# unibas-gravis/GiNGR

Measured on AMD Instinct MI355X. Metric: GiNGR update iters/sec, 50k<->50k CPD, higher is better.
Workload: dtype f64; 1 GPU; CPD update, synthetic Gaussian clouds 50000<->50000, GPMM rank 100, w=0.1, rigid global transform, sigma2_0=5032.781; points=50000, targets=50000, rank=100, parallelism=row-shard x1, exchange=single shard

## Files before the change

gingr_amd/_native.py:

```python
from __future__ import annotations

import ctypes
import os
from ctypes import POINTER, c_char_p, c_double, c_int, c_int32, c_int64, c_void_p

import numpy as np

_HERE = os.path.dirname(os.path.abspath(__file__))
LIB_PATH = os.environ.get("GINGR_HIP_LIB") or os.path.join(_HERE, "libgingr_hip.so")

GINGR_OK = 0
ERR_BAD_ARGUMENT, ERR_HIP, ERR_NONFINITE, ERR_NOT_SPD, ERR_NO_DEVICE, ERR_STATE = 1, 2, 3, 4, 5, 6
NUM_PHASES = 3
NUM_SEGMENTS = 2
SEGMENT_FULLFIT = 2
SEGMENT_REVSUM = 3
FLAVOUR_CPD, FLAVOUR_ICP, FLAVOUR_ICP_SURFACE = 0, 1, 2
RCCL_UNIQUE_ID_BYTES = 128

_STATUS_NAMES = {
    1: "GINGR_ERR_BAD_ARGUMENT", 2: "GINGR_ERR_HIP", 3: "GINGR_ERR_NONFINITE", 4: "GINGR_ERR_NOT_SPD",
    5: "GINGR_ERR_NO_DEVICE", 6: "GINGR_ERR_STATE",
}


class GingrNativeError(RuntimeError):
    def __init__(self, code: int, where: str, text: str = ""):
        self.code = code
        super().__init__(f"{where}: {_STATUS_NAMES.get(code, code)} {text}".strip())


class StateScalars(ctypes.Structure):
    _fields_ = [
        ("euler", c_double * 3), ("center", c_double * 3), ("translation", c_double * 3),
        ("scale", c_double), ("sigma2", c_double), ("iteration", c_int32), ("status", c_int32),
    ]


class CpdParams(ctypes.Structure):
    _fields_ = [("w", c_double), ("lambda_", c_double)]


class IcpParams(ctypes.Structure):
    _fields_ = [("initial_sigma", c_double), ("end_sigma", c_double), ("max_iterations", c_int32)]


class MhRequest(ctypes.Structure):
    _fields_ = [
        ("flavour", c_int32), ("kind", c_int32), ("cpd", POINTER(CpdParams)), ("icp", POINTER(IcpParams)),
        ("z", POINTER(c_double)), ("alpha", POINTER(c_double)), ("scalars", POINTER(StateScalars)),
        ("eval_sdev", c_double), ("eval_points", c_int64), ("need_forward", c_int32),
    ]


class MhResult(ctypes.Structure):
    _fields_ = [
        ("scalars", StateScalars), ("log_value", c_double), ("dist_sum", c_double), ("dist_max", c_double), ("count", c_int64),
        ("log_q_forward", c_double), ("log_q_backward", c_double), ("forward_status", c_int32), ("backward_status", c_int32),
    ]


ALLREDUCE_FN = ctypes.CFUNCTYPE(c_int, c_void_p, c_int32, c_void_p, c_int64)
_dp = POINTER(c_double)
_ip = POINTER(c_int32)

KERNEL_GAUSSIAN_MIXTURE, KERNEL_DOT, KERNEL_LOOKUP = 0, 1, 2
OPT_CULL, OPT_FINE_CULL, OPT_NN_GRID, OPT_TRI_GRID, OPT_SPLIT_EXCHANGE, OPT_GRAM_DOWNDATE = 0, 1, 2, 3, 4, 5


class ScalarKernel(ctypes.Structure):
    _fields_ = [("kind", c_int32), ("n_kernels", c_int32), ("sigmas", _dp), ("scalings", _dp), ("mirror", c_double),
                ("scaling", c_double), ("lookup", _dp)]


SIGNATURES = {
    "gingr_device_count": (c_int, []),
    "gingr_ctx_create": (c_int, [c_int, POINTER(c_void_p)]),
    "gingr_ctx_destroy": (None, [c_void_p]),
    "gingr_last_error": (c_char_p, [c_void_p]),
    "gingr_ctx_set_stream": (c_int, [c_void_p, c_void_p]),
    "gingr_ctx_get_stream": (c_void_p, [c_void_p]),
    "gingr_ctx_synchronize": (c_int, [c_void_p]),
    "gingr_build_info": (c_char_p, []),
    "gingr_ctx_set_option": (c_int, [c_void_p, c_int32, c_int32]),
    "gingr_ctx_get_option": (c_int, [c_void_p, c_int32, POINTER(c_int32)]),
    "gingr_cpd_stats": (c_int, [c_void_p, c_int64, _dp, c_int64, _dp, c_double, c_double, _dp, _dp, _dp, _dp, _dp]),
    "gingr_cpd_initial_sigma2": (c_int, [c_void_p, c_int64, _dp, c_int64, _dp, _dp]),
    "gingr_nn": (c_int, [c_void_p, c_int64, _dp, c_int64, _dp, _ip, _dp, _dp]),
    "gingr_gauss_block": (c_int, [c_void_p, c_int64, _dp, c_int64, _dp, c_double, c_double, _dp]),
    "gingr_model_upload": (c_int, [c_void_p, c_int64, c_int32, _dp, _dp, _dp, _dp, c_int64, c_int64, POINTER(c_void_p)]),
    "gingr_model_destroy": (None, [c_void_p]),
    "gingr_model_gram_exchange": (c_int, [c_void_p, POINTER(c_void_p), POINTER(c_int64)]),
    "gingr_model_finalize": (c_int, [c_void_p, c_void_p]),
    "gingr_fitter_set_meshes": (c_int, [c_void_p, c_int64, POINTER(c_int32), c_int64, POINTER(c_int32)]),
    "gingr_fitter_set_surface_method": (c_int, [c_void_p, c_int32]),
    "gingr_fitter_set_correspondence_direction": (c_int, [c_void_p, c_int32]),
    "gingr_fitter_get_reversed_correspondence": (c_int, [c_void_p, POINTER(c_int32), _dp]),
    "gingr_fitter_update_icp_surface_async": (c_int, [c_void_p, POINTER(IcpParams), c_int32]),
    "gingr_fitter_set_stop_threshold": (c_int, [c_void_p, c_double]),
    "gingr_fitter_stop_rule_hit": (c_int, [c_void_p, POINTER(c_int32)]),
    "gingr_fitter_icp_surface_phase_async": (c_int, [c_void_p, POINTER(IcpParams), c_int32]),
    "gingr_fitter_get_surface_correspondence": (c_int, [c_void_p, _dp, _dp]),
    "gingr_fitter_surface_distance_stats": (c_int, [c_void_p, c_int32, c_int64, _dp, c_int32, c_double, _dp]),
    "gingr_fitter_mh_step": (c_int, [c_void_p, POINTER(MhRequest), _dp, _dp, POINTER(MhResult)]),
    "gingr_fitter_mh_restore": (c_int, [c_void_p]),
    "gingr_classic_cpd_create": (c_int, [c_void_p, c_int32, c_int64, _dp, c_int64, _dp, c_double, c_double, c_double, POINTER(c_void_p)]),
    "gingr_classic_cpd_destroy": (None, [c_void_p]),
    "gingr_classic_cpd_iterate": (c_int, [c_void_p, c_int32]),
    "gingr_classic_cpd_get": (c_int, [c_void_p, _dp, POINTER(c_double), _dp, _dp]),
    "gingr_classic_cpd_set": (c_int, [c_void_p, _dp, c_double]),
    "gingr_mesh_distance_stats": (c_int, [c_void_p, c_int64, _dp, c_int64, _dp, c_int64, POINTER(c_int32), c_int32, c_double, _dp]),
    "gingr_fitter_update_icp_surface_sample_async": (c_int, [c_void_p, POINTER(IcpParams), _dp]),
    "gingr_fitter_posterior_logpdf_icp_surface": (c_int, [c_void_p, POINTER(IcpParams), _dp, POINTER(c_double)]),
    "gingr_rigid_icp_create": (c_int, [c_void_p, c_int32, c_int64, _dp, c_int64, _dp, POINTER(c_void_p)]),
    "gingr_rigid_icp_destroy": (None, [c_void_p]),
    "gingr_rigid_icp_iterate": (c_int, [c_void_p, c_int32, _dp]),
    "gingr_rigid_icp_get": (c_int, [c_void_p, _dp, _dp]),
    "gingr_rigid_icp_set": (c_int, [c_void_p, _dp]),
    "gingr_fitter_set_fit_points": (c_int, [c_void_p, _dp]),
    "gingr_nicp_solve": (c_int, [c_void_p, c_int32, c_int64, _dp, c_int64, _ip, _dp, _dp, c_int32, _ip, _dp, c_double, c_double, c_double,
                                 _dp, _dp]),
    "gingr_mesh_closest_points": (c_int, [c_void_p, c_int64, _dp, c_int64, _dp, c_int64, _ip, _dp, _dp, _ip, _dp]),
    "gingr_model_new_reference": (c_int, [c_void_p, c_void_p, c_int64, _dp, _ip, _dp, c_int64, c_int64, POINTER(c_void_p)]),
    "gingr_gpmm_build_diagonal": (c_int, [c_void_p, c_int64, _dp, POINTER(ScalarKernel), POINTER(ScalarKernel), POINTER(ScalarKernel),
                                          c_double, c_int32, c_int64, c_int64, POINTER(c_void_p)]),
    "gingr_gpmm_build_gaussian": (c_int, [c_void_p, c_int64, _dp, c_int32, _dp, _dp, c_double, c_int32, c_int64, c_int64,
                                          POINTER(c_void_p)]),
    "gingr_pointset_distance_extrema": (c_int, [c_void_p, _dp, c_int64, _dp, _dp]),
    "gingr_model_download": (c_int, [c_void_p, c_void_p, _dp, _dp, _dp, _dp]),
    "gingr_model_num_points": (c_int64, [c_void_p]),
    "gingr_model_rank": (c_int32, [c_void_p]),
    "gingr_model_instance": (c_int, [c_void_p, c_void_p, _dp, _dp, _dp, _dp, c_double, _dp]),
    "gingr_model_coefficients": (c_int, [c_void_p, c_void_p, _dp, _dp, _dp, _dp, _dp]),
    "gingr_model_posterior_mean": (c_int, [c_void_p, c_void_p, _dp, _dp, _dp, _dp, _dp, c_int32, _ip, _dp, _dp, _dp, _dp]),
    "gingr_fitter_create": (c_int, [c_void_p, c_void_p, POINTER(c_void_p)]),
    "gingr_fitter_destroy": (None, [c_void_p]),
    "gingr_fitter_set_target": (c_int, [c_void_p, c_int64, _dp]),
    "gingr_fitter_set_landmarks": (c_int, [c_void_p, c_int32, _ip, _dp, _dp]),
    "gingr_fitter_set_options": (c_int, [c_void_p, c_int32, c_double]),
    "gingr_fitter_set_state": (c_int, [c_void_p, _dp, POINTER(StateScalars)]),
    "gingr_fitter_get_state": (c_int, [c_void_p, _dp, POINTER(StateScalars), _dp]),
    "gingr_fitter_get_cpd_stats": (c_int, [c_void_p, _dp, _dp, _dp, _dp]),
    "gingr_fitter_get_icp_idx": (c_int, [c_void_p, _ip, _dp]),
    "gingr_fitter_update_cpd_async": (c_int, [c_void_p, POINTER(CpdParams), c_int32]),
    "gingr_fitter_update_icp_async": (c_int, [c_void_p, POINTER(IcpParams), c_int32]),
    "gingr_fitter_update_cpd_sample_async": (c_int, [c_void_p, POINTER(CpdParams), _dp]),
    "gingr_fitter_update_icp_sample_async": (c_int, [c_void_p, POINTER(IcpParams), _dp]),
    "gingr_fitter_posterior_logpdf_cpd": (c_int, [c_void_p, POINTER(CpdParams), _dp, _dp]),
    "gingr_fitter_posterior_logpdf_icp": (c_int, [c_void_p, POINTER(IcpParams), _dp, _dp]),
    "gingr_fitter_retry_counter": (c_int, [c_void_p, c_int32, POINTER(c_int32)]),
# ... 92 lines not shown
```

gingr_amd/csrc/common.h:

```cpp
#pragma once
#include <cstdlib>

#include <hip/hip_runtime.h>

#include <cstdarg>
#include <cstdint>
#include <cstdio>
#include <cstring>
#include <string>
#include <vector>

#include "../../include/gingr_hip.h"

#define GINGR_TIMERS 10

struct gingr_ctx {
    int device = 0;
    hipStream_t own_stream = nullptr;
    hipStream_t stream = nullptr;
    char err[512] = {0};
    bool timing = false;
    struct Span {
        hipEvent_t a, b;
        int which;
    };
    std::vector<Span> spans;
    std::vector<hipEvent_t> pool;
    double t_ms[GINGR_TIMERS] = {0};
    int64_t t_n[GINGR_TIMERS] = {0};
    int cull = 1;
    int tri_grid = 1;
    int nn_grid = 1;
    int32_t *regime_host = nullptr, *regime_dev = nullptr;
    int fine_override = -1;
    unsigned long long *nn_tests = nullptr;
    void *rccl_comm = nullptr;
    int32_t rccl_world = 0, rccl_rank = 0;
    int split_exchange = 0;
    int gram_downdate = -1;
    hipStream_t side_stream = nullptr, exchange_stream = nullptr;
    hipEvent_t split_ev[2] = {nullptr, nullptr};
    void *scratch = nullptr;
    size_t scratch_bytes = 0;
};

int gingr_set_error(gingr_ctx *ctx, int code, const char *fmt, ...);
void gingr_ctx_rccl_release(gingr_ctx *ctx);

#define HIP_TRY(ctx, expr)                                                                                   \
    do {                                                                                                     \
        hipError_t e__ = (expr);                                                                             \
        if (e__ != hipSuccess)                                                                               \
            return gingr_set_error((ctx), GINGR_ERR_HIP, "%s failed: %s (%s:%d)", #expr, hipGetErrorString(e__), \
                                   __FILE__, __LINE__);                                                      \
    } while (0)

#define GINGR_TRY(expr)          \
    do {                         \
        int s__ = (expr);        \
        if (s__ != GINGR_OK) return s__; \
    } while (0)

struct DevBuf {
    void *p = nullptr;
    size_t bytes = 0;
    DevBuf() = default;
    DevBuf(const DevBuf &) = delete;
    DevBuf &operator=(const DevBuf &) = delete;
    ~DevBuf() {
        if (p) (void)hipFree(p);
    }
    hipError_t alloc(size_t n) {
        if (p) (void)hipFree(p);
        p = nullptr;
        bytes = n;
        const hipError_t e = hipMalloc(&p, n ? n : 8);
        static const bool poison = getenv("GINGR_DEBUG_POISON") != nullptr;
        if (e == hipSuccess && poison) {
            (void)hipMemset(p, 0xFF, n ? n : 8);
            (void)hipDeviceSynchronize();
        }
        return e;
    }
    template <typename T>
    T *as() const {
        return reinterpret_cast<T *>(p);
    }
};

void set_dynamic_lds(const void *func, int bytes);
template <typename K>
inline void set_dynamic_lds(K *kern, size_t bytes) {
    set_dynamic_lds(reinterpret_cast<const void *>(kern), (int)bytes);
}

struct TimerScope {
    gingr_ctx *ctx;
    int which;
    hipEvent_t a = nullptr, b = nullptr;
    TimerScope(gingr_ctx *c, int w);
    void stop();
    ~TimerScope();
};

static inline int64_t ceil_div(int64_t a, int64_t b) { return (a + b - 1) / b; }
static inline int64_t round_up(int64_t a, int64_t b) { return ceil_div(a, b) * b; }

struct Cloud {
    const double *x, *y, *z;
    int64_t n;
};

int64_t cpd_colsum_ws_doubles(int64_t M, int64_t N);
int64_t cpd_rowstats_ws_doubles(int64_t M, int64_t N);
int64_t nn_ws_bytes(int64_t M, int64_t N);
bool nn_small_applies(int64_t M, int64_t N);
int64_t nn_small_ws_bytes(int64_t M, int64_t N);
void launch_nn_small(gingr_ctx *ctx, Cloud query, Cloud target, void *ws, int32_t *idx, double *d2);

#define GINGR_AUX 8
void launch_cloud_centroid(gingr_ctx *ctx, Cloud c, double *out3);
// ... 154 lines not shown
```

gingr_amd/csrc/context.hip:

```cpp
#include "common.h"

#include <map>
#include <mutex>
void set_dynamic_lds(const void *func, int bytes) {
    static std::mutex mu;
    static std::map<std::pair<int, const void *>, int> limit;
    int dev = 0;
    (void)hipGetDevice(&dev);
    std::lock_guard<std::mutex> lock(mu);
    int &have = limit[std::make_pair(dev, func)];
    if (have >= bytes) return;
    if (hipFuncSetAttribute(func, hipFuncAttributeMaxDynamicSharedMemorySize, bytes) == hipSuccess)
        have = bytes;
    else
        (void)hipGetLastError();
}


int gingr_set_error(gingr_ctx *ctx, int code, const char *fmt, ...) {
    if (ctx) {
        va_list ap;
        va_start(ap, fmt);
        vsnprintf(ctx->err, sizeof(ctx->err), fmt, ap);
        va_end(ap);
// ... 47 lines not shown
    int n = 0;
    if (hipGetDeviceCount(&n) != hipSuccess) return 0;
    return n;
}

const char *gingr_build_info(void) { return "libgingr_hip gfx950 (CDNA4) f64; built " __DATE__ " " __TIME__; }

int gingr_ctx_create(int device, gingr_ctx **out) {
    if (!out) return GINGR_ERR_BAD_ARGUMENT;
    *out = nullptr;
    int n = 0;
    if (hipGetDeviceCount(&n) != hipSuccess || n <= 0) return GINGR_ERR_NO_DEVICE;
    if (device < 0 || device >= n) return GINGR_ERR_BAD_ARGUMENT;
    if (hipSetDevice(device) != hipSuccess) return GINGR_ERR_HIP;
    gingr_ctx *ctx = new gingr_ctx();
    ctx->device = device;
    if (hipStreamCreateWithFlags(&ctx->own_stream, hipStreamNonBlocking) != hipSuccess) {
        delete ctx;
        return GINGR_ERR_HIP;
    }
    ctx->stream = ctx->own_stream;
    void *hp = nullptr, *dp = nullptr;
    if (hipHostMalloc(&hp, 64, hipHostMallocMapped) == hipSuccess) {
        memset(hp, 0, 64);
        if (hipHostGetDevicePointer(&dp, hp, 0) == hipSuccess) {
            ctx->regime_host = static_cast<int32_t *>(hp);
            ctx->regime_dev = static_cast<int32_t *>(dp);
        } else {
            (void)hipHostFree(hp);
        }
    }
    (void)hipGetLastError();
    *out = ctx;
    return GINGR_OK;
}

void gingr_ctx_destroy(gingr_ctx *ctx) {
    if (!ctx) return;
    (void)hipSetDevice(ctx->device);
    (void)hipStreamSynchronize(ctx->stream);
    timing_resolve(ctx);
    gingr_ctx_rccl_release(ctx);
    for (auto e : ctx->pool) (void)hipEventDestroy(e);
    if (ctx->scratch) (void)hipFree(ctx->scratch);
    if (ctx->nn_tests) (void)hipFree(ctx->nn_tests);
    if (ctx->regime_host) (void)hipHostFree(ctx->regime_host);
    if (ctx->side_stream) {
        (void)hipStreamSynchronize(ctx->side_stream);
        (void)hipStreamDestroy(ctx->side_stream);
    }
    for (hipEvent_t e : ctx->split_ev)
        if (e) (void)hipEventDestroy(e);
    if (ctx->own_stream) (void)hipStreamDestroy(ctx->own_stream);
    delete ctx;
}

const char *gingr_last_error(const gingr_ctx *ctx) { return ctx ? ctx->err : "null context"; }

int gingr_ctx_set_stream(gingr_ctx *ctx, void *hip_stream) {
    if (!ctx) return GINGR_ERR_BAD_ARGUMENT;
    HIP_TRY(ctx, hipStreamSynchronize(ctx->stream));
    ctx->stream = hip_stream ? reinterpret_cast<hipStream_t>(hip_stream) : ctx->own_stream;
    return GINGR_OK;
}

void *gingr_ctx_get_stream(gingr_ctx *ctx) { return ctx ? reinterpret_cast<void *>(ctx->stream) : nullptr; }

int gingr_ctx_synchronize(gingr_ctx *ctx) {
    if (!ctx) return GINGR_ERR_BAD_ARGUMENT;
    HIP_TRY(ctx, hipSetDevice(ctx->device));
    HIP_TRY(ctx, hipStreamSynchronize(ctx->stream));
    return GINGR_OK;
}

int gingr_ctx_set_option(gingr_ctx *ctx, int32_t option, int32_t value) {
    if (!ctx) return GINGR_ERR_BAD_ARGUMENT;
    switch (option) {
        case GINGR_OPT_CULL: ctx->cull = value != 0; return GINGR_OK;
        case GINGR_OPT_FINE_CULL: ctx->fine_override = value < 0 ? -1 : (value != 0); return GINGR_OK;
        case GINGR_OPT_NN_GRID: ctx->nn_grid = value < 0 ? 0 : (value > 2 ? 2 : value); return GINGR_OK;
        case GINGR_OPT_TRI_GRID: ctx->tri_grid = value < 0 ? 0 : (value > 2 ? 2 : value); return GINGR_OK;
        case GINGR_OPT_SPLIT_EXCHANGE: ctx->split_exchange = value != 0; return GINGR_OK;
        case GINGR_OPT_GRAM_DOWNDATE: ctx->gram_downdate = value < 0 ? -1 : (value != 0); return GINGR_OK;
        default: return gingr_set_error(ctx, GINGR_ERR_BAD_ARGUMENT, "ctx_set_option: unknown option %d", option);
    }
}

int gingr_ctx_get_option(gingr_ctx *ctx, int32_t option, int32_t *value) {
    if (!ctx || !value) return GINGR_ERR_BAD_ARGUMENT;
    switch (option) {
        case GINGR_OPT_CULL: *value = ctx->cull; return GINGR_OK;
        case GINGR_OPT_FINE_CULL: *value = ctx->fine_override; return GINGR_OK;
        case GINGR_OPT_NN_GRID: *value = ctx->nn_grid; return GINGR_OK;
        case GINGR_OPT_TRI_GRID: *value = ctx->tri_grid; return GINGR_OK;
        case GINGR_OPT_SPLIT_EXCHANGE: *value = ctx->split_exchange; return GINGR_OK;
        case GINGR_OPT_GRAM_DOWNDATE: *value = ctx->gram_downdate; return GINGR_OK;
        default: return gingr_set_error(ctx, GINGR_ERR_BAD_ARGUMENT, "ctx_get_option: unknown option %d", option);
    }
}

int gingr_ctx_timing_enable(gingr_ctx *ctx, int32_t enable) {
    if (!ctx) return GINGR_ERR_BAD_ARGUMENT;
    ctx->timing = enable != 0;
    return GINGR_OK;
}

int gingr_ctx_timing_read(gingr_ctx *ctx, int32_t which, double *total_ms, int64_t *launches) {
    if (!ctx || which < 0 || which >= GINGR_TIMERS) return GINGR_ERR_BAD_ARGUMENT;
    timing_resolve(ctx);
    if (total_ms) *total_ms = ctx->t_ms[which];
    if (launches) *launches = ctx->t_n[which];
    return GINGR_OK;
}

int gingr_ctx_nn_counting(gingr_ctx *ctx, int32_t enable) {
    if (!ctx) return GINGR_ERR_BAD_ARGUMENT;
    HIP_TRY(ctx, hipSetDevice(ctx->device));
    HIP_TRY(ctx, hipStreamSynchronize(ctx->stream));
    if (enable && !ctx->nn_tests) {
        void *p = nullptr;
        HIP_TRY(ctx, hipMalloc(&p, sizeof(unsigned long long)));
        ctx->nn_tests = static_cast<unsigned long long *>(p);
    }
    if (ctx->nn_tests) {
        HIP_TRY(ctx, hipMemsetAsync(ctx->nn_tests, 0, sizeof(unsigned long long), ctx->stream));
        HIP_TRY(ctx, hipStreamSynchronize(ctx->stream));
    }
    if (!enable && ctx->nn_tests) {
        (void)hipFree(ctx->nn_tests);
        ctx->nn_tests = nullptr;
    }
    return GINGR_OK;
}

int gingr_ctx_nn_tests(gingr_ctx *ctx, int64_t *tests) {
    if (!ctx || !tests) return GINGR_ERR_BAD_ARGUMENT;
    *tests = 0;
    if (!ctx->nn_tests) return gingr_set_error(ctx, GINGR_ERR_STATE, "nn_tests: counting is off (gingr_ctx_nn_counting)");
    HIP_TRY(ctx, hipSetDevice(ctx->device));
    HIP_TRY(ctx, hipStreamSynchronize(ctx->stream));
    unsigned long long v = 0;
    HIP_TRY(ctx, hipMemcpy(&v, ctx->nn_tests, sizeof(v), hipMemcpyDeviceToHost));
    *tests = (int64_t)v;
    return GINGR_OK;
}

int gingr_ctx_timing_reset(gingr_ctx *ctx) {
    if (!ctx) return GINGR_ERR_BAD_ARGUMENT;
    timing_resolve(ctx);
    for (int i = 0; i < GINGR_TIMERS; ++i) {
        ctx->t_ms[i] = 0;
        ctx->t_n[i] = 0;
    }
    return GINGR_OK;
}

}

namespace {

int upload_cloud(gingr_ctx *ctx, int64_t n, const double *host_xyz, DevBuf &staging, DevBuf &soa, Cloud *out) {
    HIP_TRY(ctx, staging.alloc((size_t)n * 3 * sizeof(double)));
    HIP_TRY(ctx, soa.alloc((size_t)n * 3 * sizeof(double)));
    HIP_TRY(ctx, hipMemcpyAsync(staging.p, host_xyz, (size_t)n * 3 * sizeof(double), hipMemcpyHostToDevice, ctx->stream));
    launch_aos_to_soa(ctx, staging.as<double>(), n, soa.as<double>());
    double *s = soa.as<double>();
    *out = Cloud{s, s + n, s + 2 * n, n};
    return GINGR_OK;
}

int check_launch(gingr_ctx *ctx) {
    HIP_TRY(ctx, hipGetLastError());
    return GINGR_OK;
}

}

extern "C" {

// ... 185 lines not shown
```

gingr_amd/csrc/fitter.hip:

```cpp
#ifdef GINGR_MH_TRACE
#include <chrono>
#include <cstdio>
#endif
#include "gp.h"

#include <algorithm>
#include <atomic>
#include <thread>
#include <chrono>
#include <cstdlib>
#include <cmath>
#include <functional>

struct gingr_fitter {
    gingr_ctx *ctx = nullptr;
    const gingr_model *m = nullptr;
    int64_t N = 0;
    double *target = nullptr;
    double *inv_den = nullptr, *Pt1 = nullptr;
    double *fit = nullptr;
    double *P1 = nullptr, *PX = nullptr;
    int32_t *nn_idx = nullptr;
    double *nn_d2 = nullptr;
    double *weight = nullptr, *evec = nullptr, *newshape = nullptr;
// ... 221 lines not shown

__global__ __launch_bounds__(256) void soa_permute_kernel(const double *__restrict__ src, const int32_t *__restrict__ perm, int64_t n,
                                                          double *__restrict__ dst) {
    const int64_t p = (int64_t)blockIdx.x * 256 + threadIdx.x;
    if (p >= n) return;
    const int64_t g = perm[p];
#pragma unroll
    for (int d = 0; d < 3; ++d) dst[d * n + p] = src[d * n + g];
}
__global__ __launch_bounds__(256) void index_map_kernel(const int32_t *__restrict__ pos, int64_t n, const int32_t *__restrict__ map,
                                                        int32_t *__restrict__ idx) {
    const int64_t j = (int64_t)blockIdx.x * 256 + threadIdx.x;
    if (j >= n) return;
    const int32_t v = pos[j];
    idx[j] = v >= 0 ? map[v] : v;
}

__global__ __launch_bounds__(256) void soa_range_kernel(const double *__restrict__ src, int64_t stride, int64_t q0, int64_t n, double *__restrict__ dst) {
    const int64_t i = (int64_t)blockIdx.x * 256 + threadIdx.x;
    if (i >= n) return;
#pragma unroll
    for (int d = 0; d < 3; ++d) dst[d * n + i] = src[d * stride + q0 + i];
}

template <typename T>
int dev_alloc(gingr_ctx *ctx, T **p, size_t count) {
    HIP_TRY(ctx, hipMalloc(reinterpret_cast<void **>(p), (count ? count : 1) * sizeof(T)));
    static const bool poison = getenv("GINGR_DEBUG_POISON") != nullptr;
    if (poison) {
        HIP_TRY(ctx, hipMemset(*p, 0xFF, (count ? count : 1) * sizeof(T)));
        HIP_TRY(ctx, hipDeviceSynchronize());
    }
    return GINGR_OK;
}

void dev_free(void *p) {
    if (p) (void)hipFree(p);
}

int check_launch(gingr_ctx *ctx) {
    HIP_TRY(ctx, hipGetLastError());
    return GINGR_OK;
}

__global__ void pose_of_state_kernel(const DevState *__restrict__ st, DevPose *__restrict__ pose) {
    const int t = threadIdx.x;
    if (t < 9) pose->R[t] = st->R[t];
    if (t < 3) {
        pose->euler[t] = st->euler[t];
        pose->t[t] = st->t[t];
        pose->center[t] = st->center[t];
    }
    if (t == 0) pose->scale = 1.0;
}

Cloud cloud_of(const double *soa, int64_t n) { return Cloud{soa, soa + n, soa + 2 * n, n}; }

int64_t split_cut(int64_t N) { return (N / 512) * 256; }

SweepArgs base_args(const gingr_fitter *f) {
    SweepArgs a;
    memset(&a, 0, sizeof(a));
    a.Q0 = f->m->Q0;
    a.ref = f->m->ref;
    a.mean = f->m->mean;
    a.M = f->m->M;
    a.rp = f->m->rp;
    a.state = f->st;
    a.pose = f->pose;
    a.c0[0] = f->m->c0[0];
    a.c0[1] = f->m->c0[1];
    a.c0[2] = f->m->c0[2];
    a.partial = f->ws;
    return a;
}

void fit_boxes_now(gingr_fitter *f) {
    if (!f->fboxes) return;
    (void)hipMemsetAsync(f->absmax + 1, 0, sizeof(double), f->ctx->stream);
    launch_tile_bbox(f->ctx, cloud_of(f->fit, f->m->M), f->fboxes, f->absmax + 2, f->absmax + 1);
    f->fit_boxes_valid = true;
}

void refresh_fit(gingr_fitter *f) {
    SweepArgs a = base_args(f);
    a.coef0 = f->alpha;
    a.shape_out = f->fit;
    if (f->fboxes && f->m->rp <= 512 && f->cpd_seen) {
        a.qboxes = f->fboxes + 6 * ceil_div(f->m->M, 256);
        a.box_centre = f->absmax + 2;
        a.absmax_slot = f->absmax + 1;
        launch_sweep(f->ctx, SWEEP_FIT, a);
        f->fit_boxes_valid = true;
    } else {
        launch_sweep(f->ctx, SWEEP_FIT, a);
        f->fit_boxes_valid = false;
        if (f->cpd_seen) fit_boxes_now(f);
    }
}

void free_meshes(gingr_fitter *f) {
    void *rptrs[] = {f->mtri_orig, f->mboundary, f->rcp, f->rd2, f->rnnd2, f->rw01, f->robs, f->rwin, f->rnn, f->rpre, f->rhit,
                     f->rkeys, f->rvals, f->rskeys, f->rsvals, f->rsort, f->radj_ptr, f->radj_tri, f->rmbnd, f->rmvn, f->rfboxes,
                     f->rtvn_loc, f->revsum, f->rws, f->gperm, f->gsorted, f->rnn_pos, f->rtri_pos};
    for (void *p : rptrs) dev_free(p);
    f->radj_ptr = f->radj_tri = f->rmbnd = nullptr;
    f->rmvn = f->rfboxes = f->rtvn_loc = f->revsum = f->gsorted = nullptr;
    f->gperm = f->rnn_pos = f->rtri_pos = nullptr;
    f->rnn_warm = f->rtri_warm = false;
    f->gather_agreed = -1;
    f->rq0 = f->rqn = 0;
    f->rws = nullptr;
    f->mtri_orig = f->mboundary = f->rnn = f->rpre = f->rhit = f->rkeys = f->rvals = f->rskeys = f->rsvals = nullptr;
    f->rcp = f->rd2 = f->rnnd2 = f->rw01 = f->robs = f->rwin = nullptr;
    f->rsort = nullptr;
    f->rsort_bytes = 0;
    f->reversed = false;
    void *ptrs[] = {f->mtri, f->ttri, f->ttri_orig, f->madj_ptr, f->madj_tri, f->tadj_ptr, f->tadj_tri, f->mcn, f->tcn, f->mvn,
                    f->tvn, f->mtboxes, f->ttboxes, f->tboundary, f->surf_cp, f->surf_d2, f->surf_w01, f->surf_win, f->surf_nnd2,
                    f->surf_nn, f->surf_pre, f->surf_hit, f->surf_tri_pos, f->mtribox, f->ttribox};
    for (void *p : ptrs) dev_free(p);
    f->mtri = f->ttri = f->ttri_orig = f->madj_ptr = f->madj_tri = f->tadj_ptr = f->tadj_tri = f->tboundary = nullptr;
    f->mcn = f->tcn = f->mvn = f->tvn = f->mtboxes = f->ttboxes = f->mtribox = f->ttribox = nullptr;
    f->surf_cp = f->surf_d2 = f->surf_w01 = f->surf_win = f->surf_nnd2 = nullptr;
    f->surf_nn = f->surf_pre = f->surf_hit = f->surf_tri_pos = nullptr;
    f->surf_tri_warm = f->surf_nn_warm = false;
    tri_grid_free(&f->ttgrid);
    mov_grid_free(&f->mgrid);
    f->Tm = f->Tt = 0;
}

int model_finalize_impl(gingr_ctx *ctx, gingr_model *m) {
    DevBuf work, flag;
    HIP_TRY(ctx, work.alloc((size_t)binv_work_doubles(m->rp) * sizeof(double)));
    HIP_TRY(ctx, flag.alloc(sizeof(int32_t)));
    launch_binv(ctx, m->r, m->rp, m->mom, work.as<double>(), m->Binv, flag.as<int32_t>());
    GINGR_TRY(check_launch(ctx));
    int32_t err = 0;
    HIP_TRY(ctx, hipMemcpyAsync(&err, flag.p, sizeof(err), hipMemcpyDeviceToHost, ctx->stream));
    HIP_TRY(ctx, hipStreamSynchronize(ctx->stream));
    if (err) return gingr_set_error(ctx, GINGR_ERR_NOT_SPD, "model finalize: Q^T Q / 1e-5 + I is not positive definite");
    const MomentLayout ml{m->rp};
    const int64_t rr = (int64_t)m->rp * m->rp;
    launch_small_gemm(ctx, m->r, m->rp, m->Binv, m->mom + ml.stot(), 1.0 / GINGR_COEFF_NOISE, m->cmat);
    for (int d = 0; d < 3; ++d)
        for (int e = 0; e < 3; ++e) {
            launch_small_gemm(ctx, m->r, m->rp, m->Binv, m->mom + ml.S(d, e), 1.0, m->cmat + (1 + d * 3 + e) * rr);
            launch_small_gemm(ctx, m->r, m->rp, m->mom + ml.S(d, e), m->cmat, 1.0, work.as<double>());
            launch_small_gemm(ctx, m->r, m->rp, m->Binv, work.as<double>(), 1.0, m->cmat + (10 + d * 3 + e) * rr);
        }
    const PostVec pvl{m->rp};
    launch_postvec(ctx, m->r, m->rp, m->Binv, m->mom + ml.V(0, 0), m->pvec);
    {
        double cst[16];
        for (int q = 0; q < 9; ++q) cst[q] = m->Pp[q];
        for (int q = 0; q < 3; ++q) {
            cst[9 + q] = m->Ps[q];
            cst[12 + q] = m->c0[q];
        }
        cst[15] = (double)m->M_total;
        HIP_TRY(ctx, hipMemcpyAsync(m->pvec + pvl.consts(), cst, sizeof(cst), hipMemcpyHostToDevice, ctx->stream));
        HIP_TRY(ctx, hipStreamSynchronize(ctx->stream));
    }
    GINGR_TRY(check_launch(ctx));
    m->eig_ready = false;
    if (m->r <= kSymEigColsMaxN) {
        if (launch_jacobi_eig(ctx, m->mom + ml.stot(), m->rp, m->r, m->eigL, m->eigV) == GINGR_OK)
            m->eig_ready = true;
        else
            (void)hipGetLastError();
    }
    HIP_TRY(ctx, hipStreamSynchronize(ctx->stream));
    m->finalized = true;
    return GINGR_OK;
}

}


int model_create_impl(gingr_ctx *ctx, int64_t M_total, int32_t rank, const double *ref, const double *mean,
                      const double *variance, int64_t row_begin, int64_t row_end,
                      const std::function<int(gingr_model *)> &fill_basis, gingr_model **out) {
    if (!ctx || !out) return GINGR_ERR_BAD_ARGUMENT;
    *out = nullptr;
    if (M_total < 1 || rank < 1 || rank > 512 || !ref || !mean || !variance)
        return gingr_set_error(ctx, GINGR_ERR_BAD_ARGUMENT, "model_upload: need M >= 1 and 1 <= rank <= 512");
    if (row_begin < 0 || row_end > M_total || row_begin >= row_end)
        return gingr_set_error(ctx, GINGR_ERR_BAD_ARGUMENT, "model_upload: bad row shard [%lld,%lld)", (long long)row_begin,
                               (long long)row_end);
    for (int32_t k = 0; k < rank; ++k)
        if (!(variance[k] >= 0.0)) return gingr_set_error(ctx, GINGR_ERR_BAD_ARGUMENT, "model_upload: variance[%d] < 0", k);
    HIP_TRY(ctx, hipSetDevice(ctx->device));
    gingr_model *m = new gingr_model();
    m->ctx = ctx;
    m->M_total = M_total;
    m->row_begin = row_begin;
    m->row_end = row_end;
    m->M = row_end - row_begin;
    m->r = rank;
    m->rp = (int32_t)round_up(rank, 16);
    m->variance.assign(variance, variance + rank);
    const int64_t M = m->M;
    double c[3] = {0, 0, 0};
    for (int64_t i = 0; i < M_total; ++i) {
        c[0] += ref[3 * i];
        c[1] += ref[3 * i + 1];
        c[2] += ref[3 * i + 2];
    }
    for (int d = 0; d < 3; ++d) m->c0[d] = c[d] / (double)M_total;

    int rc = GINGR_OK;
    DevBuf aos;
    auto fail = [&](int code) {
        gingr_model_destroy(m);
        return code;
    };
    if ((rc = dev_alloc(ctx, &m->Q0, (size_t)(3 * M + kBasisRowSlack) * m->rp)) || (rc = dev_alloc(ctx, &m->ref, (size_t)3 * M)) ||
        (rc = dev_alloc(ctx, &m->mean, (size_t)3 * M)) || (rc = dev_alloc(ctx, &m->mom, (size_t)MomentLayout{m->rp}.total())) ||
        (rc = dev_alloc(ctx, &m->Binv, (size_t)m->rp * m->rp)) || (rc = dev_alloc(ctx, &m->eigV, (size_t)m->r * m->r)) ||
        (rc = dev_alloc(ctx, &m->eigL, (size_t)m->r)) ||
        (rc = dev_alloc(ctx, &m->cmat, (size_t)19 * m->rp * m->rp)) ||
        (rc = dev_alloc(ctx, &m->pvec, (size_t)PostVec{m->rp}.total())))
        return fail(rc);
    if (aos.alloc((size_t)3 * M * sizeof(double)) != hipSuccess)
        return fail(gingr_set_error(ctx, GINGR_ERR_HIP, "model_upload: out of device memory"));
    {
        std::vector<double> pts((size_t)3 * M);
        for (int64_t i = 0; i < 3 * M; ++i) pts[(size_t)i] = ref[3 * row_begin + i] + mean[3 * row_begin + i];
        morton_order(pts.data(), M, m->hperm);
        m->hiperm.resize((size_t)M);
        for (int64_t sidx = 0; sidx < M; ++sidx) m->hiperm[(size_t)m->hperm[(size_t)sidx]] = (int32_t)sidx;
        if ((rc = dev_alloc(ctx, &m->perm, (size_t)M)) || (rc = dev_alloc(ctx, &m->iperm, (size_t)M))) return fail(rc);
        if (hipMemcpy(m->perm, m->hperm.data(), (size_t)M * sizeof(int32_t), hipMemcpyHostToDevice) != hipSuccess ||
            hipMemcpy(m->iperm, m->hiperm.data(), (size_t)M * sizeof(int32_t), hipMemcpyHostToDevice) != hipSuccess)
            return fail(gingr_set_error(ctx, GINGR_ERR_HIP, "model_upload: permutation copy failed"));
    }
    (void)hipMemsetAsync(m->Q0 + (size_t)3 * M * m->rp, 0, (size_t)kBasisRowSlack * m->rp * sizeof(double), ctx->stream);
    if ((rc = fill_basis(m))) return fail(rc);
    (void)hipMemcpyAsync(aos.p, ref + 3 * row_begin, (size_t)3 * M * sizeof(double), hipMemcpyHostToDevice, ctx->stream);
    launch_aos_to_soa(ctx, aos.as<double>(), M, m->ref, m->perm);
    (void)hipStreamSynchronize(ctx->stream);
    (void)hipMemcpyAsync(aos.p, mean + 3 * row_begin, (size_t)3 * M * sizeof(double), hipMemcpyHostToDevice, ctx->stream);
    launch_aos_to_soa(ctx, aos.as<double>(), M, m->mean, m->perm);
    {
        const MomentLayout ml{m->rp};
        DevBuf gws, sws, ptil, ev;
        if (gws.alloc((size_t)std::max(gram_ws_doubles(M, m->rp), moment_grams_ws_doubles(M, m->rp)) * sizeof(double)) != hipSuccess ||
            sws.alloc((size_t)sweep_ws_doubles(M, m->rp) * sizeof(double)) != hipSuccess ||
            ptil.alloc((size_t)3 * M * sizeof(double)) != hipSuccess || ev.alloc((size_t)3 * M * sizeof(double)) != hipSuccess)
            return fail(gingr_set_error(ctx, GINGR_ERR_HIP, "model_upload: out of device memory"));
        launch_gram(ctx, m->Q0, M, m->rp, nullptr, gws.as<double>(), m->mom + ml.stot());
        launch_moment_grams(ctx, m->Q0, M, m->rp, gws.as<double>(), m->mom);
        launch_centered_mean(ctx, m, ptil.as<double>());
        std::vector<double> ones((size_t)M, 1.0);
        DevBuf dones;
// ... 3 lines not shown
        SweepArgs a;
        memset(&a, 0, sizeof(a));
        a.Q0 = m->Q0;
        a.ref = m->ref;
        a.mean = m->mean;
        a.M = M;
        a.rp = m->rp;
        a.evec = ev.as<double>();
        a.partial = sws.as<double>();
        for (int d = 0; d < 3; ++d)
            for (int e = 0; e <= 3; ++e) {
                (void)hipMemsetAsync(ev.p, 0, (size_t)3 * M * sizeof(double), ctx->stream);
                const double *src = e < 3 ? ptil.as<double>() + (size_t)e * M : dones.as<double>();
                (void)hipMemcpyAsync(ev.as<double>() + (size_t)d * M, src, (size_t)M * sizeof(double), hipMemcpyDeviceToDevice,
                                     ctx->stream);
                a.out = m->mom + (e < 3 ? ml.V(d, e) : ml.W(d));
                launch_sweep(ctx, SWEEP_RHS, a);
            }
        if (hipGetLastError() != hipSuccess || hipStreamSynchronize(ctx->stream) != hipSuccess)
            return fail(gingr_set_error(ctx, GINGR_ERR_HIP, "model_upload: kernel launch failed"));
    }
    for (int q = 0; q < 9; ++q) m->Pp[q] = 0.0;
    for (int q = 0; q < 3; ++q) m->Ps[q] = 0.0;
    if (M != M_total) {
        m->h_full_pts.resize((size_t)3 * M_total);
        for (int64_t i = 0; i < 3 * M_total; ++i) m->h_full_pts[(size_t)i] = ref[i] + mean[i];
    }
    for (int64_t i = 0; i < M_total; ++i) {
        double pt[3];
        for (int d = 0; d < 3; ++d) pt[d] = ref[3 * i + d] + mean[3 * i + d] - m->c0[d];
        for (int d = 0; d < 3; ++d) {
            m->Ps[d] += pt[d];
            for (int e = 0; e < 3; ++e) m->Pp[d * 3 + e] += pt[d] * pt[e];
        }
    }
    if (row_begin == 0 && row_end == M_total) {
        rc = model_finalize_impl(ctx, m);
        if (rc) return fail(rc);
    }
    *out = m;
    return GINGR_OK;
}

static void free_stat_scratch(void *p);

extern "C" {

int gingr_model_upload(gingr_ctx *ctx, int64_t M_total, int32_t rank, const double *ref, const double *mean,
                       const double *basis_colmajor, const double *variance, int64_t row_begin, int64_t row_end,
                       gingr_model **out) {
    if (!ctx || !out) return GINGR_ERR_BAD_ARGUMENT;
    *out = nullptr;
    if (!basis_colmajor) return gingr_set_error(ctx, GINGR_ERR_BAD_ARGUMENT, "model_upload: basis is null");
    DevBuf stage, var;
    auto fill = [&](gingr_model *m) -> int {
        const int64_t M = m->M;
        if (stage.alloc((size_t)3 * M * rank * sizeof(double)) != hipSuccess || var.alloc(rank * sizeof(double)) != hipSuccess)
            return gingr_set_error(ctx, GINGR_ERR_HIP, "model_upload: out of device memory");
        if (hipMemcpy2DAsync(stage.p, (size_t)3 * M * sizeof(double), basis_colmajor + 3 * row_begin,
                             (size_t)3 * M_total * sizeof(double), (size_t)3 * M * sizeof(double), (size_t)rank,
                             hipMemcpyHostToDevice, ctx->stream) != hipSuccess)
            return gingr_set_error(ctx, GINGR_ERR_HIP, "model_upload: basis copy failed");
        (void)hipMemcpyAsync(var.p, variance, rank * sizeof(double), hipMemcpyHostToDevice, ctx->stream);
        launch_pack_basis(ctx, stage.as<double>(), var.as<double>(), M, rank, m->rp, m->perm, m->Q0);
        return GINGR_OK;
    };
    return model_create_impl(ctx, M_total, rank, ref, mean, variance, row_begin, row_end, fill, out);
}

void gingr_model_destroy(gingr_model *m) {
    if (!m) return;
    if (m->ctx) (void)hipSetDevice(m->ctx->device);
    dev_free(m->Q0);
    dev_free(m->ref);
    dev_free(m->mean);
    dev_free(m->mom);
    dev_free(m->Binv);
    dev_free(m->eigV);
    dev_free(m->eigL);
    dev_free(m->cmat);
    dev_free(m->pvec);
    dev_free(m->perm);
    dev_free(m->iperm);
    delete m;
}

int64_t gingr_model_num_points(const gingr_model *m) { return m ? m->M : 0; }
int32_t gingr_model_rank(const gingr_model *m) { return m ? m->r : 0; }

int gingr_model_gram_exchange(gingr_model *m, void **dev_ptr, int64_t *count) {
    if (!m || !dev_ptr || !count) return GINGR_ERR_BAD_ARGUMENT;
    *dev_ptr = m->mom;
    *count = MomentLayout{m->rp}.total();
    return GINGR_OK;
}

int gingr_model_finalize(gingr_ctx *ctx, gingr_model *m) {
    if (!ctx || !m) return GINGR_ERR_BAD_ARGUMENT;
    HIP_TRY(ctx, hipSetDevice(ctx->device));
    return model_finalize_impl(ctx, m);
}

int gingr_fitter_create(gingr_ctx *ctx, const gingr_model *model, gingr_fitter **out) {
    if (!ctx || !model || !out) return GINGR_ERR_BAD_ARGUMENT;
    *out = nullptr;
    if (!model->finalized)
        return gingr_set_error(ctx, GINGR_ERR_STATE, "fitter_create: sharded model not finalized (gingr_model_finalize)");
    HIP_TRY(ctx, hipSetDevice(ctx->device));
    gingr_fitter *f = new gingr_fitter();
    f->ctx = ctx;
    f->m = model;
    const int64_t M = model->M;
    const int32_t rp = model->rp;
    int rc;
    if ((rc = dev_alloc(ctx, &f->fit, (size_t)3 * M)) || (rc = dev_alloc(ctx, &f->P1, (size_t)M)) ||
        (rc = dev_alloc(ctx, &f->PX, (size_t)3 * M)) || (rc = dev_alloc(ctx, &f->nn_idx, (size_t)M)) ||
        (rc = dev_alloc(ctx, &f->nn_d2, (size_t)M)) || (rc = dev_alloc(ctx, &f->weight, (size_t)M)) ||
        (rc = dev_alloc(ctx, &f->zero_counts, (size_t)ceil_div(M, 256))) ||
        (rc = dev_alloc(ctx, &f->evec, (size_t)3 * M)) || (rc = dev_alloc(ctx, &f->newshape, (size_t)3 * M)) ||
        (rc = dev_alloc(ctx, &f->state_block, (size_t)rp + kScalarsDoubles + kDevStateDoubles + 8)) || (rc = dev_alloc(ctx, &f->acoef, (size_t)rp)) ||
        (rc = dev_alloc(ctx, &f->fxbuf[0], (size_t)rp * rp + 2 * rp)) || (rc = dev_alloc(ctx, &f->fxbuf[1], (size_t)rp * rp + 2 * rp)) ||
        (rc = dev_alloc(ctx, &f->nfac[0], (size_t)(rp + 16) * rp)) || (rc = dev_alloc(ctx, &f->nfac[1], (size_t)(rp + 16) * rp)) ||
        (rc = dev_alloc(ctx, &f->alt_seg, (size_t)rp * rp + 2 * rp + 8)) || (rc = dev_alloc(ctx, &f->lp_sync, (size_t)2)) ||
        (rc = dev_alloc(ctx, &f->alpha_c, (size_t)rp)) || (rc = dev_alloc(ctx, &f->zbuf, (size_t)PostVec::kZRows * rp)) || (rc = dev_alloc(ctx, &f->zrand, (size_t)rp)) ||
        (rc = dev_alloc(ctx, &f->pose, 1)) || (rc = dev_alloc(ctx, &f->fit_alt, (size_t)3 * M)) ||
        (rc = dev_alloc(ctx, &f->mh_save, (size_t)rp + kScalarsDoubles + kDevStateDoubles)) ||
        (rc = dev_alloc(ctx, &f->scalars, 8)) || (rc = dev_alloc(ctx, &f->part, GINGR_SCALAR_PART)) || (rc = dev_alloc(ctx, &f->absmax, GINGR_AUX)) || (rc = dev_alloc(ctx, &f->work, (size_t)std::max<int64_t>((int64_t)rp * rp, posterior_work_doubles(rp)))) ||
        (rc = dev_alloc(ctx, &f->lm_mask, (size_t)M))) {
        gingr_fitter_destroy(f);
        return rc;
    }
    f->alpha = f->state_block;
    f->hs_dev = reinterpret_cast<gingr_state_scalars *>(f->state_block + rp);
    f->st = reinterpret_cast<DevState *>(f->state_block + rp + kScalarsDoubles);
    f->small = f->state_block + rp + kScalarsDoubles + kDevStateDoubles;
    f->pin_doubles = (size_t)3 * M + rp + kScalarsDoubles + kDevStateDoubles + 16 + 2;
    if (hipHostMalloc(reinterpret_cast<void **>(&f->pin), f->pin_doubles * sizeof(double), hipHostMallocDefault) != hipSuccess) {
        (void)hipGetLastError();
        f->pin = nullptr;
        gingr_fitter_destroy(f);
        return gingr_set_error(ctx, GINGR_ERR_HIP, "fitter_create: pinned host buffer");
    }
    if ((rc = dev_alloc(ctx, &f->retry, 1)) || (rc = dev_alloc(ctx, &f->mh_done, 1))) {
        gingr_fitter_destroy(f);
        return rc;
    }
    f->pin[f->pin_doubles - 1] = 0.0;
    if (hipMemset(f->mh_done, 0, sizeof(int32_t)) != hipSuccess ||
        hipHostGetDevicePointer(reinterpret_cast<void **>(&f->pin_dev), f->pin, 0) != hipSuccess) {
        (void)hipGetLastError();
        f->pin_dev = nullptr;
    }
    {
        const int32_t init = GINGR_RETRY_INIT;
        if (hipMemcpy(f->retry, &init, sizeof(init), hipMemcpyHostToDevice) != hipSuccess) {
            (void)hipGetLastError();
            gingr_fitter_destroy(f);
            return gingr_set_error(ctx, GINGR_ERR_HIP, "fitter_create: retry counter upload");
        }
    }
    (void)hipMemsetAsync(f->lm_mask, 0, (size_t)M * sizeof(int32_t), ctx->stream);
    (void)hipMemsetAsync(f->alpha, 0, (size_t)rp * sizeof(double), ctx->stream);
    (void)hipMemsetAsync(f->scalars, 0, 8 * sizeof(double), ctx->stream);
    *out = f;
    return GINGR_OK;
}
// ... 716 lines not shown
                const bool alone = m->M == m->M_total && !f->partial_out;
                if (f->split_half != 0 && !alone) {
                    const int64_t NA = split_cut(tgt.n);
                    const bool first = f->split_half == 1;
                    const Cloud th = first ? Cloud{tgt.x, tgt.y, tgt.z, NA} : Cloud{tgt.x + NA, tgt.y + NA, tgt.z + NA, tgt.n - NA};
                    const int nch2 = 2 * cpd_colsum_chunks(M, tgt.n);
                    (void)launch_cpd_colsum(ctx, fit, th, &f->st->sigma2, f->absmax, f->fboxes, first ? f->ws : f->ws + (int64_t)nch2 * NA,
                                            seg0w + (first ? 0 : NA), nch2);
                    f->colsum_chunks = 0;
                    break;
                }
                f->colsum_chunks = launch_cpd_colsum(ctx, fit, tgt, &f->st->sigma2, f->absmax, f->fboxes, f->ws, alone ? nullptr : seg0w);
                if (!alone) f->colsum_chunks = 0;
            }
            break;
        }
        case 1: {
            Phase1FinalizeArgs fa;
            memset(&fa, 0, sizeof(fa));
            fa.rp = rp;
            fa.G = Gw;
            fa.rhs = rhsw;
            fa.sc8 = sc8w;
            if (icp) {
                if (f->reversed && f->sharded())
                    hipLaunchKernelGGL(reversal_local_kernel, dim3((unsigned)ceil_div(M, 256)), dim3(256), 0, ctx->stream, M, m->row_begin, m->perm,
                                       m->M_total, f->revsum, &f->st->sigma2, f->robs, f->rwin);
                if (f->reversed)
                    launch_obs_points(ctx, m, f->st, f->robs, f->rwin, f->weight, f->evec, f->lm_mask);
                else if (f->icp_surface)
                    launch_obs_points(ctx, m, f->st, f->surf_cp, f->surf_win, f->weight, f->evec, f->lm_mask, f->zero_counts);
                else if (f->n_lm != 0)
                    launch_obs_icp(ctx, m, f->st, tgt, f->nn_idx, f->lm_mask, f->weight, f->evec);
                fa.scalar_mode = 0;
            } else {
                launch_cpd_den_finalize(ctx, tgt, &f->st->sigma2, cp->w, m->M_total, seg0, f->inv_den, f->Pt1, f->tile_bad, f->part,
                                        f->scalars, f->colsum_chunks > 0 ? f->ws : nullptr, f->colsum_chunks);
                f->colsum_chunks = 0;
                CpdObsArgs ob;
                memset(&ob, 0, sizeof(ob));
                ob.ref = m->ref;
                ob.mean = m->mean;
                ob.sigma2 = &f->st->sigma2;
                ob.R = f->st->R;
                ob.center = f->st->center;
                ob.t = f->st->t;
                ob.lambda = cp->lambda;
                ob.lm_mask = f->lm_mask;
                ob.weight = f->weight;
                ob.evec = f->evec;
                launch_cpd_rowstats(ctx, fit, tgt, &f->st->sigma2, f->absmax, f->inv_den, f->tboxes, f->tile_bad, f->ws, f->P1,
                                    f->PX, f->part, f->scalars, nullptr, 0, &ob, false);
                fa.scalar_mode = 1;
                fa.part = f->part;
                fa.scalars_local = f->scalars;
                fa.contribute_xpx = m->row_begin == 0 ? 1 : 0;
            }
            double *gram_ws = f->ws, *sweep_ws = f->ws + gram_ws_doubles(M, rp);
            bool rhs_done = false;
            ZeroGate rhs_gate{};
            if (icp && !f->icp_surface && !f->reversed && f->n_lm == 0) {
                fa.nslabs = 0;
                fa.scaled_src = m->mom + MomentLayout{rp}.stot();
                fa.sigma2 = &f->st->sigma2;
                fa.scaled_contribute = m->row_begin == 0 ? 1 : 0;
            } else if (icp && f->icp_surface && !f->reversed &&
                       (ctx->gram_downdate == 1 || (ctx->gram_downdate < 0 && M >= kGramDowndateMinRows))) {
                const bool gated = ctx->gram_downdate != 1;
                ZeroGate few{f->zero_counts, (int32_t)ceil_div(M, 256), 0, M}, many = few;
                many.run_if_many = 1;
                fa.gram_partial = gram_ws;
                fa.nslabs = launch_gram_downdate(ctx, m->Q0, M, rp, f->weight, gram_ws, gated ? &few : nullptr);
                fa.scaled_src = m->mom + MomentLayout{rp}.stot();
                fa.sigma2 = &f->st->sigma2;
                fa.scaled_contribute = m->row_begin == 0 ? 1 : 0;
                if (gated) {
                    bool alt_rhs = false;
                    fa.alt_nslabs = launch_gram(ctx, m->Q0, M, rp, f->weight, gram_ws, nullptr, f->evec, sweep_ws, &alt_rhs, &many);
                    fa.gate = many;
                    rhs_gate = few;
                }
            } else {
                fa.gram_partial = gram_ws;
                fa.nslabs = launch_gram(ctx, m->Q0, M, rp, f->weight, gram_ws, nullptr, f->evec, sweep_ws, &rhs_done);
            }
            fa.sweep_partial = sweep_ws;
            if (rhs_done) {
                fa.sweep_blocks = fa.nslabs;
            } else {
                SweepArgs a = base_args(f);
                a.evec = f->evec;
                a.partial = sweep_ws;
                a.no_reduce = 1;
                a.gate = rhs_gate;
                if (icp && !f->icp_surface && !f->reversed && f->n_lm == 0) {
                    a.state = f->st;
                    a.icp_idx = f->nn_idx;
                    a.tx = tgt.x, a.ty = tgt.y, a.tz = tgt.z;
                    a.n_targets = tgt.n;
                    a.lm_mask = f->lm_mask;
                    a.weight_out = f->weight, a.evec_out = f->evec;
                    launch_sweep(ctx, SWEEP_RHS_ICP, a);
                } else {
                    launch_sweep(ctx, SWEEP_RHS, a);
                }
                fa.sweep_blocks = sweep_num_blocks(M);
            }
            launch_phase1_finalize(ctx, fa);
            launch_landmarks(ctx, m, f->st, f->n_lm, f->lm_pid, f->lm_xyz, f->lm_cov, Gw, rhsw);
            break;
        }
        case 2: {
            const bool eig = icp && !f->icp_surface && !f->reversed && f->n_lm == 0 && !f->zrand_active && m->eig_ready;
            if (eig)
                launch_posterior_solve_eig(ctx, r, rp, m->eigV, m->eigL, &f->st->sigma2, rhs, f->acoef, f->st);
            else if (f->zrand_active && f->allow_alt && f->post_stage == 2 && f->nf_valid[f->live] && m->M == m->M_total && !f->partial_out)
                launch_posterior_sample_cached(ctx, r, rp, f->nfac[f->live], f->fxbuf[f->live] + (int64_t)rp * rp, f->zrand, f->acoef, f->st);
            else
                launch_posterior_solve(ctx, r, rp, G, rhs, f->zrand_active ? f->zrand : nullptr, f->work, f->acoef, f->st);
            launch_post_matvecs(ctx, m, f->alpha, f->acoef, f->zbuf);
            PostSolveArgs a;
            memset(&a, 0, sizeof(a));
            a.r = r;
            a.rp = rp;
            a.pvec = m->pvec;
            a.zbuf = f->zbuf;
            a.alpha = f->alpha;
            a.scalars = sc8;
            a.is_icp = icp ? 1 : 0;
            if (icp) {
                a.icp_step = (ip->initial_sigma - ip->end_sigma) / (double)ip->max_iterations;
                a.icp_end = ip->end_sigma;
            }
            a.step = f->step_length;
            a.global_transform = f->global_transform;
            a.state = f->st;
            a.retry = f->retry;
            a.zero_slot = f->absmax + 1;
            a.probabilistic = f->zrand_active ? 1 : 0;
            a.stop_threshold = f->stop_threshold;
            launch_post_solve(ctx, a);
            refresh_fit(f);
            break;
        }
        default:
            return gingr_set_error(ctx, GINGR_ERR_BAD_ARGUMENT, "phase %d out of range", phase);
    }
    return check_launch(ctx);
}

int check_ready(gingr_fitter *f) {
    if (!f) return GINGR_ERR_BAD_ARGUMENT;
    if (!f->target) return gingr_set_error(f->ctx, GINGR_ERR_STATE, "update: no target set (gingr_fitter_set_target)");
    if (!f->has_state) return gingr_set_error(f->ctx, GINGR_ERR_STATE, "update: no state set (gingr_fitter_set_state)");
    if (hipSetDevice(f->ctx->device) != hipSuccess) return gingr_set_error(f->ctx, GINGR_ERR_HIP, "hipSetDevice failed");
    return GINGR_OK;
}

}

extern "C" {

int gingr_fitter_cpd_phase_async(gingr_fitter *f, const gingr_cpd_params *p, int32_t phase) {
    GINGR_TRY(check_ready(f));
    if (!p || !(p->w >= 0.0 && p->w < 1.0) || !(p->lambda > 0.0))
        return gingr_set_error(f->ctx, GINGR_ERR_BAD_ARGUMENT, "cpd params: need 0 <= w < 1 and lambda > 0");
    return run_phase(f, false, p, nullptr, phase);
}

int gingr_fitter_icp_phase_async(gingr_fitter *f, const gingr_icp_params *p, int32_t phase) {
    GINGR_TRY(check_ready(f));
    if (!p || p->max_iterations < 1) return gingr_set_error(f->ctx, GINGR_ERR_BAD_ARGUMENT, "icp params: max_iterations < 1");
    f->icp_surface = false;
    return run_phase(f, true, nullptr, p, phase);
}

int gingr_fitter_update_cpd_async(gingr_fitter *f, const gingr_cpd_params *p, int32_t n_iterations) {
    GINGR_TRY(check_ready(f));
    if (f->m->M != f->m->M_total)
        return gingr_set_error(f->ctx, GINGR_ERR_STATE, "update_cpd_async: sharded model needs the phase API + exchange");
    for (int32_t it = 0; it < n_iterations; ++it) {
        TimerScope ts(f->ctx, 3);
        for (int ph = 0; ph < GINGR_NUM_PHASES; ++ph) GINGR_TRY(gingr_fitter_cpd_phase_async(f, p, ph));
    }
    return GINGR_OK;
}

int gingr_fitter_update_icp_async(gingr_fitter *f, const gingr_icp_params *p, int32_t n_iterations) {
    GINGR_TRY(check_ready(f));
    if (f->m->M != f->m->M_total)
        return gingr_set_error(f->ctx, GINGR_ERR_STATE, "update_icp_async: sharded model needs the phase API + exchange");
    for (int32_t it = 0; it < n_iterations; ++it) {
        TimerScope ts(f->ctx, 3);
        for (int ph = 0; ph < GINGR_NUM_PHASES; ++ph) GINGR_TRY(gingr_fitter_icp_phase_async(f, p, ph));
    }
    return GINGR_OK;
}

}

// ... 1321 lines not shown
```

gingr_amd/csrc/gp.h:

```cpp
#pragma once

#include "common.h"
#include "svd3.h"

#include <functional>

#define GINGR_COEFF_NOISE 1e-5

struct DevState {
    double R[9];
    double euler[3];
    double center[3];
    double t[3];
    double scale;
    double sigma2;
    int32_t iteration;
    int32_t status;
    int32_t err;
    int32_t pad;
    int32_t stopped;
    int32_t pad2;
};

__device__ inline void state_init_body(DevState *st, const gingr_state_scalars *h, double *zero_slot) {
    if (zero_slot) *zero_slot = 0.0;
    for (int q = 0; q < 3; ++q) {
        st->euler[q] = h->euler[q];
        st->center[q] = h->center[q];
        st->t[q] = h->translation[q];
    }
    euler_to_rot(st->euler, st->R);
    st->scale = h->scale;
    st->sigma2 = h->sigma2;
    st->iteration = h->iteration;
    st->status = h->status;
    st->err = 0;
    st->pad = 0;
    st->stopped = 0;
    st->pad2 = 0;
}

struct DevPose {
    double R[9];
    double euler[3];
    double t[3];
    double center[3];
    double scale;
};

struct MomentLayout {
    int32_t rp;
    __host__ __device__ int64_t stot() const { return 0; }
    __host__ __device__ int64_t S(int d, int e) const { return (int64_t)rp * rp * (1 + d * 3 + e); }
    __host__ __device__ int64_t V(int d, int e) const { return (int64_t)rp * rp * 10 + (int64_t)rp * (d * 3 + e); }
    __host__ __device__ int64_t W(int d) const { return (int64_t)rp * rp * 10 + (int64_t)rp * (9 + d); }
    __host__ __device__ int64_t total() const { return (int64_t)rp * rp * 10 + (int64_t)rp * 12; }
};

struct PostVec {
    int32_t rp;
    static constexpr int kV = 0;
    static constexpr int kW = 9;
    static constexpr int kBV = 12;
    static constexpr int kBW = 21;
    static constexpr int kRows = 24;
    __host__ __device__ int64_t consts() const { return (int64_t)kRows * rp; }
    __host__ __device__ int64_t total() const { return consts() + 16; }
    static constexpr int kZa = 0;
    static constexpr int kBSa = 9;
    static constexpr int kBTa = 18;
    static constexpr int kA1 = 27;
    static constexpr int kZRows = 28;
};

constexpr int kBasisRowSlack = 144;

struct gingr_model {
    gingr_ctx *ctx = nullptr;
    int64_t M_total = 0, row_begin = 0, row_end = 0, M = 0;
    int32_t r = 0, rp = 0;
    double *Q0 = nullptr;
    double *ref = nullptr;
    double *mean = nullptr;
    double *mom = nullptr;
    int32_t *perm = nullptr;
    std::vector<int32_t> hperm, hiperm;
    int32_t *iperm = nullptr;
    std::vector<double> h_full_pts;
    double *Binv = nullptr;
    double *eigV = nullptr;
    double *eigL = nullptr;
    bool eig_ready = false;
    double *cmat = nullptr;
    double *pvec = nullptr;
    double c0[3] = {0, 0, 0};
    double Pp[9] = {0};
    double Ps[3] = {0};
    std::vector<double> variance;
    bool finalized = false;
};

void launch_interp_pack(gingr_ctx *ctx, const double *Qs, int32_t rp, const int32_t *inv_src, const int32_t *ids, const double *w,
                        const int32_t *perm_new, int64_t row_begin, int64_t M, double *Q0);

int model_create_impl(gingr_ctx *ctx, int64_t M_total, int32_t rank, const double *ref, const double *mean,
                      const double *variance, int64_t row_begin, int64_t row_end,
                      const std::function<int(gingr_model *)> &fill_basis, gingr_model **out);

void fitter_set_partial_output(gingr_fitter *f, double *base);
void fitter_set_partial_fullfit(gingr_fitter *f, double *base);
typedef int (*fitter_gather_fn)(void *user, gingr_fitter *f);
int fitter_sharded_update(gingr_fitter *f, int flavour, const gingr_cpd_params *cp, const gingr_icp_params *ip, int32_t n_iterations,
                          const double *z, gingr_allreduce_fn reduce, void *user, fitter_gather_fn gather = nullptr, bool split_native = false);
int fitter_sharded_logpdf(gingr_fitter *f, int flavour, const gingr_cpd_params *cp, const gingr_icp_params *ip, const double *mesh_xyz_full,
                          gingr_allreduce_fn reduce, void *user, double *logpdf, fitter_gather_fn gather = nullptr);
int fitter_run_phase(gingr_fitter *f, int flavour, const gingr_cpd_params *cp, const gingr_icp_params *ip, int phase);
int fitter_logpdf_prepare(gingr_fitter *f, const double *mesh_xyz_full);
int fitter_logpdf_finish(gingr_fitter *f, double *logpdf);
int fitter_set_zrand(gingr_fitter *f, const double *z);
double *fitter_fullfit(gingr_fitter *f);
void fitter_set_partial_revsum(gingr_fitter *f, double *base);
double *fitter_revsum(gingr_fitter *f);
gingr_ctx *fitter_ctx(gingr_fitter *f);
bool fitter_gather_possible(gingr_fitter *f, int32_t world, int32_t rank);
int fitter_gather_agreed(gingr_fitter *f, int32_t world);
void fitter_set_gather_agreed(gingr_fitter *f, int32_t world, int agreed);
const gingr_model *fitter_model(gingr_fitter *f);

struct ZeroGate {
    const int32_t *counts;
    int32_t nblocks;
    int32_t run_if_many;
    int64_t M;
};

__device__ __forceinline__ bool gate_open(const ZeroGate &g) {
    if (!g.counts) return true;
    __shared__ int gate_sum;
    if (threadIdx.x == 0) gate_sum = 0;
    __syncthreads();
    int s = 0;
    for (int b = threadIdx.x; b < g.nblocks; b += blockDim.x) s += g.counts[b];
#pragma unroll
    for (int off = 32; off > 0; off >>= 1) s += __shfl_xor(s, off);
    if ((threadIdx.x & 63) == 0 && s != 0) atomicAdd(&gate_sum, s);
    __syncthreads();
    const bool many = (int64_t)gate_sum * 8 > g.M;
    return many == (g.run_if_many != 0);
}

enum SweepMode {
    SWEEP_RHS = 0,
    SWEEP_PROJ1 = 1,
    SWEEP_SHAPES = 2,
    SWEEP_PROJ2 = 3,
    SWEEP_FIT = 4,
    SWEEP_POSED = 5,
    SWEEP_RHS_ICP = 6
};

struct SweepArgs {
    const double *Q0;
    const double *ref;
    const double *mean;
    int64_t M;
    int32_t rp;
    const double *coef0;
    const double *coef1;
    const double *evec;
    const double *shape_in;
    double *shape_out;
    const DevState *state;
    const DevPose *pose;
    double c0[3];
    double *partial;
    double *out;
    double *zero_slot;
    double *qboxes;
    const double *box_centre;
    double *absmax_slot;
    int32_t no_reduce;
    const int32_t *icp_idx;
    const double *tx, *ty, *tz;
    int64_t n_targets;
    const int32_t *lm_mask;
    double *weight_out, *evec_out;
    const DevState *frame;
    ZeroGate gate;
};

int sweep_num_blocks(int64_t M);
int64_t sweep_ws_doubles(int64_t M, int32_t rp);
void launch_sweep(gingr_ctx *ctx, SweepMode mode, const SweepArgs &a);

int64_t gram_ws_doubles(int64_t M, int32_t rp);
int launch_gram(gingr_ctx *ctx, const double *Q0, int64_t M, int32_t rp, const double *weight, double *ws, double *G,
                const double *evec = nullptr, double *rhs_partial = nullptr, bool *rhs_done = nullptr, const ZeroGate *gate = nullptr);

int64_t gram_wide_ws_doubles(int64_t M, int32_t rp);
int launch_gram_wide(gingr_ctx *ctx, const double *Q0, int64_t M, int32_t rp, const double *weight, double *ws, const double *evec,
                     double *rhs_partial, const ZeroGate *gate = nullptr);

int64_t gram_rows_ws_doubles(int64_t rows, int32_t rp);
int launch_gram_rows(gingr_ctx *ctx, const double *Z, int64_t rows, int32_t rp, double *ws);

struct Phase1FinalizeArgs {
    int32_t rp;
    const double *gram_partial;
    int32_t nslabs;
    const double *scaled_src;
    const double *sigma2;
    int32_t scaled_contribute;
    double *G;
    const double *sweep_partial;
    int32_t sweep_blocks;
    double *rhs;
    int32_t scalar_mode;
    const double *part;
    double *scalars_local;
    double *sc8;
    int32_t contribute_xpx;
    ZeroGate gate;
    int32_t alt_nslabs;
};
void launch_phase1_finalize(gingr_ctx *ctx, const Phase1FinalizeArgs &a);
int launch_gram_downdate(gingr_ctx *ctx, const double *Q0, int64_t M, int32_t rp, const double *weight, double *ws,
                         const ZeroGate *gate = nullptr);

void launch_obs_cpd(gingr_ctx *ctx, const gingr_model *m, const DevState *st, Cloud fit, const double *P1,
                    const double *PX, double lambda, const int32_t *lm_mask, double *weight, double *evec);
void launch_obs_icp(gingr_ctx *ctx, const gingr_model *m, const DevState *st, Cloud target, const int32_t *idx,
                    const int32_t *lm_mask, double *weight, double *evec);
void launch_obs_points(gingr_ctx *ctx, const gingr_model *m, const DevState *st, const double *obs_soa,
                       const double *weight_in, double *weight, double *evec, const int32_t *lm_mask = nullptr,
                       int32_t *zero_counts = nullptr);
void launch_landmarks(gingr_ctx *ctx, const gingr_model *m, const DevState *st, int32_t n_lm, const int32_t *lm_pid_local,
                      const double *lm_xyz, const double *lm_cov, double *G, double *rhs);

void launch_posterior_solve(gingr_ctx *ctx, int32_t r, int32_t rp, const double *G, const double *rhs, const double *zrand,
                            double *work, double *a, DevState *st);
int launch_posterior_logpdf(gingr_ctx *ctx, int32_t r, int32_t rp, const double *G, const double *rhs, const double *Stot,
                            const double *qte, double *fx, bool cached, double *work, double *out2, unsigned *sync = nullptr,
                            unsigned epoch = 0, bool keep_factor = true, double *nfac = nullptr);
void launch_posterior_sample_cached(gingr_ctx *ctx, int32_t r, int32_t rp, const double *nfac, const double *a_mean, const double *zrand,
                                    double *a, DevState *st);
void launch_posterior_solve_eig(gingr_ctx *ctx, int32_t r, int32_t rp, const double *eigV, const double *eigL, const double *sigma2,
                                const double *rhs, double *a, DevState *st);
int launch_jacobi_eig(gingr_ctx *ctx, const double *G, int32_t ldg, int32_t n, double *evals, double *Vs);
constexpr int kSymEigColsMaxN = 192;
int64_t sym_eig_cols_work_doubles(int32_t n);
void launch_sym_eig_cols(gingr_ctx *ctx, int count, const double *const *G, const int32_t *ldg, const int32_t *n, double *const *work,
                         double *const *evals, double *const *Vs, int32_t *const *info);
int64_t posterior_work_doubles(int32_t rp);
int64_t binv_work_doubles(int32_t rp);
void launch_binv(gingr_ctx *ctx, int32_t r, int32_t rp, const double *S, double *work, double *Binv, int32_t *err_flag);
void launch_coeff_solve(gingr_ctx *ctx, int32_t r, int32_t rp, const double *Binv, const double *p, double *out);
void launch_state_init(gingr_ctx *ctx, DevState *st, const gingr_state_scalars *host_scalars_dev, double *zero_slot = nullptr);

int64_t moment_grams_ws_doubles(int64_t M, int32_t rp);
void launch_moment_grams(gingr_ctx *ctx, const double *Q0, int64_t M, int32_t rp, double *ws, double *mom);
void launch_centered_mean(gingr_ctx *ctx, const gingr_model *m, double *ptil);

struct PostSolveArgs {
    int32_t r, rp;
    const double *pvec;
    const double *zbuf;
    double *alpha;
    const double *scalars;
    int32_t is_icp;
    double icp_step, icp_end;
    double step;
    int32_t global_transform;
    DevState *state;
    double *zero_slot;
    int32_t *retry;
    int32_t probabilistic;
    double stop_threshold;
};
#define GINGR_RETRY_INIT 10
void launch_post_solve(gingr_ctx *ctx, const PostSolveArgs &a);
void launch_post_matvecs(gingr_ctx *ctx, const gingr_model *m, const double *alpha, const double *a, double *zbuf);
void launch_small_gemm(gingr_ctx *ctx, int32_t r, int32_t rp, const double *A, const double *B, double scale, double *out);
void launch_postvec(gingr_ctx *ctx, int32_t r, int32_t rp, const double *Binv, const double *moment_vectors, double *pvec);

void launch_pack_basis(gingr_ctx *ctx, const double *stage_colmajor, const double *variance_dev, int64_t M, int32_t r,
                       int32_t rp, const int32_t *perm, double *Q0);
```

gingr_amd/csrc/gp.hip:

```cpp
#include "gp.h"
#include "svd3.h"

#include <algorithm>
#include <type_traits>

namespace {

typedef double v4f64 __attribute__((ext_vector_type(4)));


__device__ __forceinline__ bool finite_d(double v) { return fabs(v) <= 1.79769313486231570815e308; }

__global__ __launch_bounds__(256) void interp_pack_kernel(const double *__restrict__ Qs, int32_t rp, const int32_t *__restrict__ inv_src,
                                                          const int32_t *__restrict__ ids, const double *__restrict__ w,
                                                          const int32_t *__restrict__ perm_new, int64_t row_begin, int64_t M,
                                                          double *__restrict__ Q0) {
    const int64_t idx = (int64_t)blockIdx.x * 256 + threadIdx.x;
    if (idx >= 3 * M * rp) return;
    const int64_t row = idx / rp;
    const int32_t q = (int32_t)(idx - row * rp);
    const int64_t s = row / 3;
    const int d = (int)(row - 3 * s);
    const int64_t o = row_begin + perm_new[s];
    double acc = 0.0;
// ... 156 lines not shown
                a.shape_out[p] = nx;
                a.shape_out[M + p] = ny;
                a.shape_out[2 * M + p] = nz;
                const double x0 = rx + mx + f1[0] - a.c0[0], x1 = ry + my + f1[1] - a.c0[1], x2 = rz + mz + f1[2] - a.c0[2];
                const double y0 = nx - a.c0[0], y1 = ny - a.c0[1], y2 = nz - a.c0[2];
                us[0] += x0; us[1] += x1; us[2] += x2;
                us[3] += y0; us[4] += y1; us[5] += y2;
                us[6] += y0 * x0; us[7] += y0 * x1; us[8] += y0 * x2;
                us[9] += y1 * x0; us[10] += y1 * x1; us[11] += y1 * x2;
                us[12] += y2 * x0; us[13] += y2 * x1; us[14] += y2 * x2;
                us[15] += x0 * x0 + x1 * x1 + x2 * x2;
            }
        } else if (MODE == SWEEP_PROJ2) {
            const double sx = a.shape_in[pc] - cen[0] - tr[0], sy = a.shape_in[M + pc] - cen[1] - tr[1],
                         sz = a.shape_in[2 * M + pc] - cen[2] - tr[2];
            e[0] = R[0] * sx + R[3] * sy + R[6] * sz - (rx - cen[0]) - mx;
            e[1] = R[1] * sx + R[4] * sy + R[7] * sz - (ry - cen[1]) - my;
            e[2] = R[2] * sx + R[5] * sy + R[8] * sz - (rz - cen[2]) - mz;
        } else if (MODE == SWEEP_FIT || MODE == SWEEP_POSED) {
            const double ix = rx + mx + f0[0] - cen[0], iy = ry + my + f0[1] - cen[1], iz = rz + mz + f0[2] - cen[2];
            const double nx = R[0] * ix + R[1] * iy + R[2] * iz + cen[0] + tr[0];
            const double ny = R[3] * ix + R[4] * iy + R[5] * iz + cen[1] + tr[1];
            const double nz = R[6] * ix + R[7] * iy + R[8] * iz + cen[2] + tr[2];
            if (valid && lane16 == 0) {
                const double s = (MODE == SWEEP_FIT) ? scale : 1.0;
                a.shape_out[p] = s * nx;
                a.shape_out[M + p] = s * ny;
                a.shape_out[2 * M + p] = s * nz;
            }
        }
        if (TRANS) {
            if (!valid) e[0] = e[1] = e[2] = 0.0;
#pragma unroll
            for (int m = 0; m < KMAX; ++m) {
                if (m < km) {
                    const int k = m * 16;
                    acc[m] = __builtin_fma(q0[k], e[0], __builtin_fma(q1[k], e[1], __builtin_fma(q2[k], e[2], acc[m])));
                }
            }
        }
    }
    if (TRANS) {
        __syncthreads();
#pragma unroll
        for (int m = 0; m < KMAX; ++m)
            if (m < km) red[grp * rp + m * 16 + lane16] = acc[m];
        __syncthreads();
        for (int k = tid; k < rp; k += kSweepThreads) {
            double s = 0.0;
            for (int g = 0; g < kGroups; ++g) s += red[g * rp + k];
            a.partial[(int64_t)blockIdx.x * rp + k] = s;
        }
    }
    if (MODE == SWEEP_SHAPES) {
        __syncthreads();
        if (lane16 == 0)
            for (int s = 0; s < 16; ++s) red[grp * 16 + s] = us[s];
        __syncthreads();
        if (tid < 24) {
            double s = 0.0;
            if (tid < 16)
                for (int g = 0; g < kGroups; ++g) s += red[g * 16 + tid];
            a.partial[(int64_t)blockIdx.x * 24 + tid] = s;
        }
    }
}

__global__ __launch_bounds__(256) void block_partials_reduce_kernel(const double *__restrict__ partial, int nblocks, int width,
                                                                    double *__restrict__ out) {
    __shared__ double sh[256];
    const int k = blockIdx.x;
    double s = 0.0;
    for (int b = threadIdx.x; b < nblocks; b += 256) s += partial[(int64_t)b * width + k];
    sh[threadIdx.x] = s;
    __syncthreads();
#pragma unroll
    for (int st = 128; st > 0; st >>= 1) {
        if ((int)threadIdx.x < st) sh[threadIdx.x] += sh[threadIdx.x + st];
        __syncthreads();
    }
    if (threadIdx.x == 0) out[k] = sh[0];
}

template <int KM, int S>
__global__ __launch_bounds__(kSweepThreads) void sweep_fit_boxes_kernel(SweepArgs a) {
    constexpr int CH = KM < 8 ? KM : 8;
    static_assert(4 % S == 0, "points per group and round");
    extern __shared__ double lds[];
    const int tid = threadIdx.x, lane16 = tid & 15, grp = tid >> 4;
    const int rp = a.rp, km = rp >> 4;
    const int64_t M = a.M;
    double *coef = lds, *red = lds + rp;
    for (int k = tid; k < rp; k += kSweepThreads) coef[k] = a.coef0[k];
    double R[9], tr[3], cen[3];
    for (int q = 0; q < 9; ++q) R[q] = a.state->R[q];
    for (int q = 0; q < 3; ++q) {
        tr[q] = a.state->t[q];
        cen[q] = a.state->center[q];
    }
    const double scale = a.state->scale;
    double cf[KM];
    __syncthreads();
#pragma unroll
    for (int m = 0; m < KM; ++m) cf[m] = m < km ? coef[m * 16 + lane16] : 0.0;
    double amax = 0.0;
    for (int64_t qd = blockIdx.x; qd * 64 < M; qd += gridDim.x) {
        double lo[3] = {__builtin_huge_val(), __builtin_huge_val(), __builtin_huge_val()};
        double hi[3] = {-__builtin_huge_val(), -__builtin_huge_val(), -__builtin_huge_val()};
#pragma unroll
        for (int s0 = 0; s0 < 4; s0 += S) {
            double facc[S][3], rm[S][3];
#pragma unroll
            for (int s = 0; s < S; ++s)
#pragma unroll
                for (int d = 0; d < 3; ++d) facc[s][d] = 0.0;
#pragma unroll
            for (int mc = 0; mc < KM; mc += CH) {
                double u[S][3][CH];
#pragma unroll
                for (int s = 0; s < S; ++s) {
                    const int64_t p = qd * 64 + (s0 + s) * kGroups + grp;
                    const int64_t pc = p < M ? p : 0;
                    const double *q0 = a.Q0 + (3 * pc) * rp + lane16;
#pragma unroll
                    for (int d = 0; d < 3; ++d) {
#pragma unroll
                        for (int m = 0; m < CH; ++m) u[s][d][m] = (mc + m < KM && mc + m < km) ? q0[d * rp + (mc + m) * 16] : 0.0;
                        if (mc == 0) rm[s][d] = a.ref[d * M + pc] + a.mean[d * M + pc];
                    }
                }
#pragma unroll
                for (int s = 0; s < S; ++s)
#pragma unroll
                    for (int d = 0; d < 3; ++d)
#pragma unroll
                        for (int m = 0; m < CH; ++m)
                            if (mc + m < KM) facc[s][d] = __builtin_fma(u[s][d][m], cf[mc + m], facc[s][d]);
            }
#pragma unroll
            for (int s = 0; s < S; ++s) {
                const int64_t p = qd * 64 + (s0 + s) * kGroups + grp;
                double f[3];
#pragma unroll
                for (int d = 0; d < 3; ++d) f[d] = group16_sum(facc[s][d]);
                const double ix = rm[s][0] + f[0] - cen[0], iy = rm[s][1] + f[1] - cen[1], iz = rm[s][2] + f[2] - cen[2];
                const double nx = scale * (R[0] * ix + R[1] * iy + R[2] * iz + cen[0] + tr[0]);
                const double ny = scale * (R[3] * ix + R[4] * iy + R[5] * iz + cen[1] + tr[1]);
                const double nz = scale * (R[6] * ix + R[7] * iy + R[8] * iz + cen[2] + tr[2]);
                if (p < M) {
                    if (lane16 == 0) {
                        a.shape_out[p] = nx;
                        a.shape_out[M + p] = ny;
                        a.shape_out[2 * M + p] = nz;
                    }
                    lo[0] = fmin(lo[0], nx), lo[1] = fmin(lo[1], ny), lo[2] = fmin(lo[2], nz);
                    hi[0] = fmax(hi[0], nx), hi[1] = fmax(hi[1], ny), hi[2] = fmax(hi[2], nz);
                }
            }
        }
        if (lane16 == 0) {
#pragma unroll
            for (int d = 0; d < 3; ++d) {
                red[grp * 8 + d] = lo[d];
                red[grp * 8 + 3 + d] = hi[d];
            }
        }
        __syncthreads();
        if (tid < 6) {
            double v = red[tid];
            for (int g = 1; g < kGroups; ++g) v = tid < 3 ? fmin(v, red[g * 8 + tid]) : fmax(v, red[g * 8 + tid]);
            a.qboxes[qd * 6 + tid] = v;
            red[kGroups * 8 + tid] = fabs(v - a.box_centre[tid % 3]);
        }
        __syncthreads();
        if (tid == 0)
            for (int q = 0; q < 6; ++q) amax = fmax(amax, red[kGroups * 8 + q]);
        __syncthreads();
    }
    if (tid == 0 && a.absmax_slot) {
        const unsigned long long mb = __builtin_bit_cast(unsigned long long, amax);
        if (mb > __hip_atomic_load(reinterpret_cast<unsigned long long *>(a.absmax_slot), __ATOMIC_RELAXED, __HIP_MEMORY_SCOPE_AGENT))
            atomicMax(reinterpret_cast<unsigned long long *>(a.absmax_slot), mb);
    }
}

__global__ __launch_bounds__(256) void gram_kernel(const double *__restrict__ Q0, int64_t rows, int rp,
                                                   const double *__restrict__ weight, int64_t rows_per_slab, int nbp,
                                                   int row_stride, int offA, int offB, int full,
                                                   double *__restrict__ partial) {
    __shared__ double red[16 * 4 * 64];
    int pa = 0, pb = 0;
    if (full) {
        pa = blockIdx.y / nbp;
        pb = blockIdx.y - pa * nbp;
    } else {
        int t = blockIdx.y;
        for (pa = 0; pa < nbp; ++pa) {
            const int cnt = nbp - pa;
            if (t < cnt) {
                pb = pa + t;
                break;
            }
            t -= cnt;
        }
    }
    const int wave = threadIdx.x >> 6, lane = threadIdx.x & 63, kq = lane >> 4, cl = lane & 15;
    const int64_t r0 = (int64_t)blockIdx.x * rows_per_slab;
    const int64_t r1 = min(rows, r0 + rows_per_slab);
    v4f64 acc[4][4];
#pragma unroll
    for (int i = 0; i < 4; ++i)
#pragma unroll
        for (int j = 0; j < 4; ++j) acc[i][j] = v4f64{0, 0, 0, 0};
    const bool vla = pa * 64 + 4 * cl < rp, vlb = pb * 64 + 4 * cl < rp;
    const bool diag = pa == pb && offA == offB;
    typedef double d4 __attribute__((ext_vector_type(4)));
    double ca[4], cb[4];
    auto load = [&](int64_t row, double fa[4], double fb[4]) {
        const int64_t rr = row + kq;
        const bool valid = rr < r1;
// ... 4 lines not shown
#pragma unroll
        for (int t = 0; t < 4; ++t) fb[t] = vb4[t];
        if (diag) {
#pragma unroll
            for (int t = 0; t < 4; ++t) fa[t] = fb[t] * wv;
        } else {
            d4 va4 = d4{0, 0, 0, 0};
            if (vla && valid) va4 = *reinterpret_cast<const d4 *>(Q0 + (rc * row_stride + offA) * rp + pa * 64 + 4 * cl);
#pragma unroll
            for (int t = 0; t < 4; ++t) fa[t] = va4[t] * wv;
        }
    };
    int64_t row = r0 + 4 * wave;
    if (row < r1) load(row, ca, cb);
    for (; row < r1; row += 16) {
        double na[4] = {0, 0, 0, 0}, nb[4] = {0, 0, 0, 0};
        if (row + 16 < r1) load(row + 16, na, nb);
#pragma unroll
        for (int i = 0; i < 4; ++i)
#pragma unroll
            for (int j = 0; j < 4; ++j) acc[i][j] = __builtin_amdgcn_mfma_f64_16x16x4f64(ca[i], cb[j], acc[i][j], 0, 0, 0);
#pragma unroll
        for (int t = 0; t < 4; ++t) {
            ca[t] = na[t];
            cb[t] = nb[t];
        }
    }
    for (int w = 1; w < 4; ++w) {
        __syncthreads();
        if (wave == w) {
#pragma unroll
            for (int i = 0; i < 4; ++i)
#pragma unroll
                for (int j = 0; j < 4; ++j)
#pragma unroll
                    for (int reg = 0; reg < 4; ++reg) red[((i * 4 + j) * 4 + reg) * 64 + lane] = acc[i][j][reg];
        }
        __syncthreads();
        if (wave == 0) {
#pragma unroll
            for (int i = 0; i < 4; ++i)
#pragma unroll
                for (int j = 0; j < 4; ++j)
#pragma unroll
                    for (int reg = 0; reg < 4; ++reg) acc[i][j][reg] += red[((i * 4 + j) * 4 + reg) * 64 + lane];
        }
    }
    if (wave != 0) return;
    double *out = partial + (int64_t)blockIdx.x * rp * rp;
#pragma unroll
    for (int i = 0; i < 4; ++i)
#pragma unroll
        for (int j = 0; j < 4; ++j) {
#pragma unroll
            for (int reg = 0; reg < 4; ++reg) {
                const int gi = pa * 64 + 4 * (kq + 4 * reg) + i;
                const int gj = pb * 64 + 4 * cl + j;
                if (gi < rp && gj < rp) out[(int64_t)gi * rp + gj] = acc[i][j][reg];
            }
        }
}

template <int BEGIN, int END, typename F>
__device__ __forceinline__ void static_for(F &&f) {
    if constexpr (BEGIN < END) {
        f(std::integral_constant<int, BEGIN>{});
        static_for<BEGIN + 1, END>(f);
    }
}

template <int NT>
__host__ __device__ constexpr int tri_row(int q) {
    int t = 0;
    while (q >= NT - t) q -= NT - t, ++t;
    return t;
}
template <int NT>
__host__ __device__ constexpr int tri_col(int q) {
    int t = 0;
    while (q >= NT - t) q -= NT - t, ++t;
    return t + q;
}

template <int NT, int HALF, bool FULL>
__device__ __forceinline__ void gram_tri_half(const double *__restrict__ Q0, int rp, const double *__restrict__ weight, int64_t r0,
                                              int64_t r1, int kgroup, int kq, int cl, int lane, double *red, double *xchg,
                                              double *__restrict__ out, const double *__restrict__ evec, int64_t npts,
                                              double *__restrict__ rhs_out, double *rsh) {
    constexpr int kTiles = NT * (NT + 1) / 2;
    constexpr int kMine = HALF == 0 ? (kTiles + 1) / 2 : kTiles / 2;
    constexpr int kM = kMine > 0 ? kMine : 1;
    v4f64 acc[kM];
#pragma unroll
    for (int q = 0; q < kMine; ++q) acc[q] = v4f64{0, 0, 0, 0};
    constexpr int kOwn = HALF == 0 ? (NT + 1) / 2 : NT / 2;
    constexpr int kO = kOwn > 0 ? kOwn : 1;
    const bool with_rhs = evec != nullptr;
    const bool with_w = weight != nullptr;
    const int kgu = __builtin_amdgcn_readfirstlane(kgroup);
    const int64_t ubase = r0 + 4 * kgu;
    const int64_t first = ubase + kq;
    const double *pclamp = Q0 + r0 * rp + cl;
    const double *pnext = Q0 + first * rp + cl;
    const int64_t pstep = 16 * (int64_t)rp;
    int64_t left_u = r1 - ubase;
    const int64_t pt_first = first / 3;
    const int rem_first = (int)(first - 3 * pt_first);
    constexpr unsigned kThird = 0x55555556u;
    unsigned third = (unsigned)rem_first * kThird;
    const double *wclamp = with_w ? weight + r0 / 3 : pclamp;
    const double *eclamp = with_rhs ? evec + r0 / 3 : pclamp;
    const double *wp = with_w ? weight + pt_first : pclamp;
    const double *ep = with_rhs ? evec + rem_first * npts + pt_first : pclamp;
    const int64_t estep = with_rhs ? 5 + npts : 0, ewrap = with_rhs ? 6 - 2 * npts : 0;
    double fn[2][kO], wn[2], en[2];
    int vrows[2];
    auto load_next = [&](auto slot) __attribute__((always_inline)) {
        constexpr int L = decltype(slot)::value;
        if (left_u >= 4) {
            vrows[L] = 4;
#pragma unroll
            for (int k = 0; k < kOwn; ++k) fn[L][k] = pnext[16 * (2 * k + HALF)];
            wn[L] = *wp;
            en[L] = *ep;
        } else {
            vrows[L] = (int)max((int64_t)0, left_u);
            const bool valid = left_u > kq;
            const double *p = valid ? pnext : pclamp;
#pragma unroll
            for (int k = 0; k < kOwn; ++k) fn[L][k] = p[16 * (2 * k + HALF)];
            wn[L] = *(valid ? wp : wclamp);
            en[L] = *(valid ? ep : eclamp);
        }
        left_u -= 16;
        pnext += pstep;
        const unsigned t2 = third + kThird;
        const bool wrap = t2 < third;
        third = t2;
        wp += wrap ? 6 : 5;
        ep += wrap ? ewrap : estep;
    };
    double racc[kO];
#pragma unroll
    for (int k = 0; k < kOwn; ++k) racc[k] = 0.0;
    const int64_t nsteps = (r1 - r0 + 15) / 16;
    constexpr int kBufStride = 4 * 2 * NT * 64;
    double *xbuf = xchg + (size_t)kgu * 2 * NT * 64 + lane;
    double cur[2][NT], a[2][NT];
    auto hand_over_write = [&](auto slot) __attribute__((always_inline)) {
        constexpr int L = decltype(slot)::value;
        double w = wn[L], e = en[L];
        if constexpr (!FULL) {
            w = with_w ? w : 1.0;
            e = with_rhs ? e : 0.0;
        }
        if (vrows[L] < 4) {
            asm volatile("; rows past the slab");
            const bool valid = vrows[L] > kq;
            w = valid ? w : 0.0;
            e = valid ? e : 0.0;
        }
#pragma unroll
        for (int k = 0; k < kOwn; ++k) {
            xbuf[L * kBufStride + (2 * k + HALF) * 64] = fn[L][k];
            xbuf[L * kBufStride + (NT + 2 * k + HALF) * 64] = fn[L][k] * w;
            racc[k] = __builtin_fma(fn[L][k], e, racc[k]);
        }
    };
    auto hand_over_read = [&](auto set) __attribute__((always_inline)) {
        constexpr int S = decltype(set)::value;
#pragma unroll
        for (int t = 0; t < NT; ++t) {
            cur[S][t] = xbuf[S * kBufStride + t * 64];
            a[S][t] = xbuf[S * kBufStride + (NT + t) * 64];
        }
    };
    auto mfmas = [&](auto set, auto begin, auto endq) __attribute__((always_inline)) {
        constexpr int S = decltype(set)::value;
        static_for<decltype(begin)::value, decltype(endq)::value>([&](auto m) {
            constexpr int mi = decltype(m)::value, q = 2 * mi + HALF, tr = tri_row<NT>(q), tc = tri_col<NT>(q);
            acc[mi] = __builtin_amdgcn_mfma_f64_16x16x4f64(a[S][tr], cur[S][tc], acc[mi], 0, 0, 0);
        });
    };
    using std::integral_constant;
    constexpr integral_constant<int, 0> c0{};
    constexpr integral_constant<int, 1> c1{};
    constexpr int kQ1 = kMine / 4, kQ2 = kMine / 2, kQ3 = (3 * kMine) / 4;
    load_next(c0);
    load_next(c1);
    hand_over_write(c0);
    __syncthreads();
    load_next(c0);
    hand_over_read(c0);
    auto step = [&](auto set) __attribute__((always_inline)) {
        constexpr int S = decltype(set)::value, T = 1 - S;
        constexpr integral_constant<int, T> other{};
        __builtin_amdgcn_sched_barrier(0);
        mfmas(set, integral_constant<int, 0>{}, integral_constant<int, kQ1>{});
        __builtin_amdgcn_sched_barrier(0);
        hand_over_write(other);
        __builtin_amdgcn_sched_barrier(0);
        mfmas(set, integral_constant<int, kQ1>{}, integral_constant<int, kQ2>{});
        __builtin_amdgcn_sched_barrier(0);
        __syncthreads();
        load_next(other);
        hand_over_read(other);
        __builtin_amdgcn_sched_barrier(0);
        mfmas(set, integral_constant<int, kQ2>{}, integral_constant<int, kQ3>{});
        __builtin_amdgcn_sched_barrier(0);
        mfmas(set, integral_constant<int, kQ3>{}, integral_constant<int, kMine>{});
        __builtin_amdgcn_sched_barrier(0);
    };
    int64_t st = 0;
    for (; st + 1 < nsteps; st += 2) {
        step(c0);
        step(c1);
    }
    if (st < nsteps) step(c0);
    __syncthreads();
    if (evec) {
#pragma unroll
        for (int k = 0; k < kOwn; ++k) {
            racc[k] += __shfl_xor(racc[k], 16);
            racc[k] += __shfl_xor(racc[k], 32);
        }
        if (kq == 0)
#pragma unroll
            for (int k = 0; k < kOwn; ++k) rsh[kgroup * (NT * 16) + (2 * k + HALF) * 16 + cl] = racc[k];
        __syncthreads();
        if (HALF == 0 && kgroup == 0 && kq == 0)
#pragma unroll
            for (int t = 0; t < NT; ++t) {
                const int c = t * 16 + cl;
                rhs_out[c] = ((rsh[c] + rsh[NT * 16 + c]) + rsh[2 * NT * 16 + c]) + rsh[3 * NT * 16 + c];
            }
    }
    static_assert(((kTiles + 1) / 2) * 2 * 256 <= 2 * kBufStride, "the exchange area must hold one slot of the K-group reduction");
    double *slot0 = red + HALF * ((kTiles + 1) / 2) * 256, *slot1 = xchg + HALF * ((kTiles + 1) / 2) * 256;
    auto put = [&](double *slot) {
#pragma unroll
        for (int q = 0; q < kMine; ++q)
#pragma unroll
            for (int reg = 0; reg < 4; ++reg) slot[(q * 4 + reg) * 64 + lane] = acc[q][reg];
    };
    auto add = [&](const double *slot) {
#pragma unroll
        for (int q = 0; q < kMine; ++q)
#pragma unroll
            for (int reg = 0; reg < 4; ++reg) acc[q][reg] += slot[(q * 4 + reg) * 64 + lane];
    };
    if (kgroup >= 2) put(kgroup == 2 ? slot0 : slot1);
    __syncthreads();
    if (kgroup < 2) add(kgroup == 0 ? slot0 : slot1);
    __syncthreads();
    if (kgroup == 1) put(slot0);
    __syncthreads();
    if (kgroup == 0) add(slot0);
    if (kgroup != 0) return;
    int q = 0;
#pragma unroll
    for (int t = 0; t < NT; ++t)
#pragma unroll
        for (int u = t; u < NT; ++u, ++q)
            if ((q & 1) == HALF)
#pragma unroll
                for (int reg = 0; reg < 4; ++reg) out[(int64_t)(16 * t + kq + 4 * reg) * rp + 16 * u + cl] = acc[q >> 1][reg];
}

template <int NT, bool FULL>
__global__ __launch_bounds__(512) void gram_tri_kernel(const double *__restrict__ Q0, int64_t rows, int rp,
                                                       const double *__restrict__ weight, int64_t rows_per_slab,
                                                       double *__restrict__ partial, const double *__restrict__ evec, int64_t npts,
                                                       double *__restrict__ rhs_partial, ZeroGate gate) {
    constexpr int kTiles = NT * (NT + 1) / 2;
    if (!gate_open(gate)) return;
    __shared__ double red[(kTiles + 1) * 256];
    __shared__ double xchg[2 * 4 * 2 * NT * 64];
    __shared__ double rsh[4 * NT * 16];
    const int wave = threadIdx.x >> 6, lane = threadIdx.x & 63, kq = lane >> 4, cl = lane & 15;
    const int64_t r0 = (int64_t)blockIdx.x * rows_per_slab;
    const int64_t r1 = min(rows, r0 + rows_per_slab);
    double *out = partial + (int64_t)blockIdx.x * rp * rp;
    double *rhs_out = rhs_partial ? rhs_partial + (int64_t)blockIdx.x * rp : nullptr;
    if ((wave >> 2) == 0)
        gram_tri_half<NT, 0, FULL>(Q0, rp, weight, r0, r1, wave & 3, kq, cl, lane, red, xchg, out, evec, npts, rhs_out, rsh);
    else
        gram_tri_half<NT, 1, FULL>(Q0, rp, weight, r0, r1, wave & 3, kq, cl, lane, red, xchg, out, evec, npts, rhs_out, rsh);
}

__global__ __launch_bounds__(256) void gram_reduce_kernel(const double *__restrict__ partial, int nslabs, int rp, int symmetric,
                                                          double *__restrict__ G) {
    __shared__ double sh[8][33];
    const int el = threadIdx.x & 31, g = threadIdx.x >> 5;
    const int idx = blockIdx.x * 32 + el;
    const int rr = rp * rp;
    const int i = idx / rp, j = idx - i * rp;
    const bool need = idx < rr && !(symmetric && i > j);
    double s = 0.0;
    if (need) {
        const double *p = partial + idx;
#pragma unroll 8
        for (int b = g; b < nslabs; b += 8) s += p[(int64_t)b * rr];
    }
    sh[g][el] = s;
    __syncthreads();
    if (g == 0 && need) {
        const double t = ((sh[0][el] + sh[1][el]) + (sh[2][el] + sh[3][el])) + ((sh[4][el] + sh[5][el]) + (sh[6][el] + sh[7][el]));
        G[i * rp + j] = t;
        if (symmetric) G[j * rp + i] = t;
    }
}

__global__ __launch_bounds__(256) void phase1_finalize_kernel(Phase1FinalizeArgs A) {
    __shared__ double sh[8][33];
    __shared__ double sv[256];
    const int rp = A.rp, rr = rp * rp;
    const int nG = (A.nslabs > 0 || A.scaled_src) ? (rr + 31) / 32 : 0;
    const int b = blockIdx.x;
    if (A.gate.counts && gate_open(A.gate)) {
        A.nslabs = A.alt_nslabs;
        A.scaled_src = nullptr;
        A.sweep_blocks = A.alt_nslabs;
    }
    if (b < nG) {
        const int el = threadIdx.x & 31, g = threadIdx.x >> 5;
        const int idx = b * 32 + el;
        if (A.nslabs <= 0) {
            if (g == 0 && idx < rr) A.G[idx] = A.scaled_contribute ? A.scaled_src[idx] * (1.0 / A.sigma2[0]) : 0.0;
            return;
        }
        const int i = idx / rp, j = idx - i * rp;
        const bool need = idx < rr && !(i > j);
        double s = 0.0;
        if (need) {
            const double *p = A.gram_partial + idx;
#pragma unroll 8
            for (int q = g; q < A.nslabs; q += 8) s += p[(int64_t)q * rr];
        }
        sh[g][el] = s;
        __syncthreads();
        if (g == 0 && need) {
            double t = ((sh[0][el] + sh[1][el]) + (sh[2][el] + sh[3][el])) + ((sh[4][el] + sh[5][el]) + (sh[6][el] + sh[7][el]));
            if (A.scaled_src)
                t = ((A.scaled_contribute ? A.scaled_src[idx] : 0.0) - t) * (1.0 / A.sigma2[0]);
            A.G[i * rp + j] = t;
            A.G[j * rp + i] = t;
        }
        return;
    }
    if (b < nG + rp) {
        const int k = b - nG;
        double s = 0.0;
        for (int q = threadIdx.x; q < A.sweep_blocks; q += 256) s += A.sweep_partial[(int64_t)q * rp + k];
        sv[threadIdx.x] = s;
        __syncthreads();
#pragma unroll
        for (int st = 128; st > 0; st >>= 1) {
            if ((int)threadIdx.x < st) sv[threadIdx.x] += sv[threadIdx.x + st];
            __syncthreads();
        }
        if (threadIdx.x == 0) A.rhs[k] = sv[0];
        return;
    }
    if (A.scalar_mode == 1) {
        const int map[4] = {1, 0, 2, 3};
        for (int q = 0; q < 4; ++q) {
            sv[threadIdx.x] = A.part[q * GINGR_SCALAR_BLOCKS + threadIdx.x];
            __syncthreads();
#pragma unroll
            for (int st = 128; st > 0; st >>= 1) {
                if ((int)threadIdx.x < st) sv[threadIdx.x] += sv[threadIdx.x + st];
                __syncthreads();
            }
            if (threadIdx.x == 0) {
                const double tot = sv[0];
                if (A.scalars_local) A.scalars_local[map[q]] = tot;
                A.sc8[map[q]] = (map[q] == 1 && !A.contribute_xpx) ? 0.0 : tot;
            }
            __syncthreads();
        }
        if (threadIdx.x >= 4 && threadIdx.x < 8) A.sc8[threadIdx.x] = 0.0;
    } else if (threadIdx.x < 8) {
        A.sc8[threadIdx.x] = 0.0;
    }
}

__global__ __launch_bounds__(256) void gram_downdate_kernel(const double *__restrict__ Q0, int64_t M, int rp, const double *__restrict__ weight,
                                                            int64_t verts_per_slab, double *__restrict__ partial, ZeroGate gate) {
    if (!gate_open(gate)) return;
    constexpr int kBatch = 4;
    int pa = 0, pb = 0;
    {
        const int np = (rp + 111) / 112;
        int t = blockIdx.y;
        for (pa = 0; pa < np; ++pa) {
            if (t < np - pa) {
                pb = pa + t;
                break;
            }
            t -= np - pa;
        }
    }
    const int ca0 = 112 * pa, cb0 = 112 * pb;
    __shared__ double q[kBatch][3][112], qb[kBatch][3][112];
    __shared__ unsigned long long zmask[16];
// ... 633 lines not shown
    GINGR_STAGE_CLOCK(4)
    GINGR_STAGE_CLOCK(6)
#endif
}

constexpr int kSolveThreads = 256;

template <bool FAST, typename PtrD>
__device__ __forceinline__ void posterior_solve_body(PtrD sm, int r, int rp, const double *__restrict__ G, const double *__restrict__ rhs,
                                                     const double *__restrict__ zrand, double *__restrict__ a, DevState *__restrict__ st,
                                                     int *bad_spd, int *bad) {
    const int n = rp, ld = solve_ld(n);
    constexpr int XR = FAST ? 2 * kNB : kNB;
    auto A = sm;
    auto y = sm + (size_t)n * ld;
    auto rd = sm + (size_t)(n + XR) * ld;
    auto y2 = rd + n;
    const int tid = threadIdx.x;
    if (tid == 0) {
        *bad_spd = 0;
        *bad = 0;
    }
    for (int k = tid; k < kNB * ld; k += kSolveThreads) y[k] = k < r ? rhs[k] : 0.0;
    for (int k = tid; k < n; k += kSolveThreads) y2[k] = (zrand && k < r) ? zrand[k] : 0.0;
    if (FAST)
        for (int k = tid; k < kNB * ld; k += kSolveThreads) {
            const int c = k / ld, j = k - c * ld;
            y[kNB * ld + k] = (j < n && (j & 15) == c) ? 1.0 : 0.0;
        }
    GINGR_STAGE_CLOCK(7)
    lds_load_spd<kSolveThreads>(A, ld, r, n, G, 1.0, nullptr, 0.0, 1.0);
    GINGR_STAGE_CLOCK(0)
    lds_cholesky<kSolveThreads>(A, ld, n, rd, bad_spd, kNB, FAST ? kNB : 0);
    GINGR_STAGE_CLOCK(4)
    if constexpr (FAST) {
        if (zrand) {
            lds_backward_w<kSolveThreads>(A, ld, n, y + kNB * ld, y2, rd);
            for (int k = tid; k < n; k += kSolveThreads) y2[k] = rd[k];
            __syncthreads();
        }
        lds_backward_w<kSolveThreads>(A, ld, n, y + kNB * ld, y, rd);
        for (int k = tid; k < n; k += kSolveThreads) y[k] = rd[k];
        __syncthreads();
    } else {
        lds_backward<kSolveThreads>(A, ld, n, rd, y);
        if (zrand) lds_backward<kSolveThreads>(A, ld, n, rd, y2);
    }
    GINGR_STAGE_CLOCK(5)
    GINGR_STAGE_CLOCK(6)
    for (int k = tid; k < rp; k += kSolveThreads) {
        const double v = k < r ? y[k] + y2[k] : 0.0;
        a[k] = v;
        if (!finite_d(v)) *bad = 1;
    }
    __syncthreads();
    if (tid == 0) {
        if (*bad_spd)
            st->err = GINGR_ERR_NOT_SPD;
        else if (*bad)
            st->err = GINGR_ERR_NONFINITE;
    }
}

template <int MODE>
__global__ __launch_bounds__(kSolveThreads) void posterior_solve_lds_kernel(int r, int rp, const double *__restrict__ G,
                                                                  const double *__restrict__ rhs,
                                                                  const double *__restrict__ zrand, double *__restrict__ a,
                                                                  DevState *__restrict__ st, double *gwork) {
    extern __shared__ double lds_sm[];
    __shared__ int bad_spd, bad;
#ifdef GINGR_SOLVE_TWICE
    for (int pass = 0; pass < 2; ++pass) {
        __syncthreads();
#endif
    if constexpr (MODE == 2)
        posterior_solve_body<false>(gwork, r, rp, G, rhs, zrand, a, st, &bad_spd, &bad);
    else
        posterior_solve_body<MODE == 0>(lds_sm, r, rp, G, rhs, zrand, a, st, &bad_spd, &bad);
#ifdef GINGR_SOLVE_TWICE
    }
#endif
}

constexpr int kWideSolveThreads = 512;

template <int SW>
struct WideSolveLds {
    double rdl[SW];
    double red[2][kWideSolveThreads / 64][SW];
    double xs[2][512];
    double yv[2][SW];
    int bad_spd;
};

template <int SW, bool HAS_S>
__device__ __forceinline__ void wide_solve_body(double *P, WideSolveLds<SW> &Ls, int r, int n, const double *__restrict__ G, double ca,
                                                const double *__restrict__ S, double cs, double ci, const double *__restrict__ b1,
                                                const double *__restrict__ b2, double cb, const double *__restrict__ zrand, double *gw) {
    constexpr int ldp = SW + 1, NW = kWideSolveThreads / 64;
    double *rdl = Ls.rdl;
    auto &red = Ls.red;
    auto &xs = Ls.xs;
    auto &yv = Ls.yv;
    int &bad_spd = Ls.bad_spd;
    const int tid = threadIdx.x, lane = tid & 63, wave = tid >> 6, l15 = lane & 15, l4 = lane >> 4;
    double *Lg = gw;
    double *rdg = gw + (size_t)(n + kNB) * n;
    const int nvec = zrand ? 2 : 1;
    if (tid == 0) bad_spd = 0;
    GINGR_STAGE_CLOCK(7)
    typedef double d2 __attribute__((ext_vector_type(2)));
    constexpr int NTJ = SW / 16;
    constexpr int TSTEP = NW / NTJ;
    constexpr int TACC = SW == 64 ? 9 : 9;
    constexpr int HALF = SW / 2;
    constexpr int RSTEP = kWideSolveThreads / HALF;
    constexpr int PRE = 17;
    const int wv = __builtin_amdgcn_readfirstlane(wave);
    const int my_tj = wv % NTJ, ti0 = wv / NTJ;
    for (int e = tid; e < kNB * n; e += kWideSolveThreads) Lg[(size_t)n * n + e] = e < r ? (b2 ? __builtin_fma(cb, b2[e], b1[e]) : b1[e]) : 0.0;
    __syncthreads();
    const int srow = tid / HALF, scp = tid % HALF;
    for (int kb = 0; kb < n; kb += SW) {
        const int sw = min(SW, n - kb), rows = n - kb + kNB;
        const int nti = rows >> 4, ntj = sw >> 4;
        v4f64 acc[TACC];
#pragma unroll
        for (int q = 0; q < TACC; ++q) acc[q] = v4f64{0, 0, 0, 0};
        const bool col_live = my_tj < ntj;
        const int nsl = kb / SW;
        d2 pre[PRE];
        auto fetch_slice = [&](int sl) __attribute__((always_inline)) {
            const bool is_c = sl == nsl;
            const int col = sl * SW + 2 * scp;
            const double *base = (is_c ? G : Lg) + col;
#pragma unroll
            for (int u = 0; u < PRE; ++u) {
                const int gi = kb + srow + u * RSTEP;
                if (gi < n + kNB) pre[u] = *reinterpret_cast<const d2 *>((gi < n ? base : Lg + col) + (size_t)gi * n);
            }
            if (is_c) {
                d2 ps[HAS_S ? PRE : 1];
                if (HAS_S) {
#pragma unroll
                    for (int u = 0; u < PRE; ++u) {
                        const int gi = kb + srow + u * RSTEP;
                        if (gi < n) ps[u] = *reinterpret_cast<const d2 *>(S + col + (size_t)gi * n);
                    }
                }
#pragma unroll
                for (int u = 0; u < PRE; ++u) {
                    const int gi = kb + srow + u * RSTEP;
                    if (gi < n) {
#pragma unroll
                        for (int h = 0; h < 2; ++h) {
                            const double one = gi == col + h ? 1.0 : 0.0;
                            double t = ca * pre[u][h];
                            if (HAS_S) t = __builtin_fma(cs, ps[u][h], t);
                            pre[u][h] = (gi < r && col + h < r) ? t + ci * one : one;
                        }
                    }
                }
            }
        };
        fetch_slice(0);
        for (int sl = 0; sl <= nsl; ++sl) {
// ... 877 lines not shown
            for (int b = 0; b < 3; ++b) {
                p[6 + d * 3 + b] = V[b * 3 + d] * al;
                p[15 + d * 3 + b] = V[d * 3 + b] * ac;
                p[24 + d * 3 + b] = ac * za[d * 3 + b];
            }
        }
    }
    if (tid == 0) bad = 0;
    __syncthreads();
    if (tid < 144) {
        const int t = tid >> 2, part = tid & 3;
        const double *colp = prod + part * ld + t;
        double s = 0.0;
        for (int k = 0; k < rp; k += 4) s += colp[k * ld];
        s += __shfl_xor(s, 1);
        s += __shfl_xor(s, 2);
        if (part == 0) L.D[t] = s;
    }
    __syncthreads();
    if (tid < 64) post_pose_step(A, st, A.pvec + pvl.consts(), L, &bad);
    __syncthreads();
    double anew = 0.0;
    if (tid < rp) {
        double s = 0.0;
#pragma unroll
        for (int q = 0; q < 9; ++q) {
            s = __builtin_fma(L.coef[q], BV[q], s);
            s = __builtin_fma(L.coef[9 + q], bz[q], s);
        }
#pragma unroll
        for (int d = 0; d < 3; ++d) s = __builtin_fma(L.coef[18 + d], BW[d], s);
        anew = tid < r ? s / GINGR_COEFF_NOISE : 0.0;
        if (!finite_d(anew)) bad = 1;
    }
    __syncthreads();
    const bool posterior_failed = st->err != 0;
    const bool failed = posterior_failed || bad != 0;
    const double sigma2_before = st->sigma2;
    __syncthreads();
    if (!failed) {
        if (tid < rp) A.alpha[tid] = anew;
        if (tid < 20) reinterpret_cast<double *>(st)[tid] = L.stage[tid];
    }
    if (tid == 0) {
        if (posterior_failed) {
            if (st->iteration > 0) {
                if (A.probabilistic && A.retry && *A.retry > 0)
                    *A.retry -= 1;
                else
                    st->status = GINGR_FIT_MODEL_FLEXIBILITY_ERROR;
            }
        } else {
            if (A.retry) *A.retry = *A.retry + 1 < GINGR_RETRY_INIT ? *A.retry + 1 : GINGR_RETRY_INIT;
            if (bad != 0) st->status = GINGR_FIT_MODEL_FLEXIBILITY_ERROR;
        }
        st->pad = failed ? (st->err != 0 ? st->err : GINGR_ERR_NONFINITE) : 0;
        st->err = 0;
        st->iteration += 1;
        if (A.stop_threshold >= 0.0 && fabs(sigma2_before - (failed ? sigma2_before : L.stage[19])) < A.stop_threshold) st->stopped = 1;
    }
}

__global__ void state_init_kernel(DevState *st, const gingr_state_scalars *h, double *zero_slot) {
    if (threadIdx.x != 0 || blockIdx.x != 0) return;
    state_init_body(st, h, zero_slot);
}

}

int sweep_num_blocks(int64_t M) {
    const int64_t nb = ceil_div(M, kGroups);
    return (int)(nb < kSweepMaxBlocks ? (nb > 0 ? nb : 1) : kSweepMaxBlocks);
}

int64_t sweep_ws_doubles(int64_t M, int32_t rp) {
    const int w = rp > 24 ? rp : 24;
    return (int64_t)sweep_num_blocks(M) * w;
}

template <int MODE>
static void launch_sweep_mode(gingr_ctx *ctx, const SweepArgs &a, int width) {
    if (MODE == SWEEP_FIT && a.qboxes && a.rp <= 512) {
        const int nq = (int)std::min<int64_t>(4096, ceil_div(a.M, 64));
        const size_t l2 = (size_t)(a.rp + kGroups * 8 + 8) * sizeof(double);
        TimerScope ts(ctx, 4);
        if (a.rp <= 64)
            hipLaunchKernelGGL((sweep_fit_boxes_kernel<4, 4>), dim3(nq), dim3(kSweepThreads), l2, ctx->stream, a);
        else if (a.rp <= 112)
            hipLaunchKernelGGL((sweep_fit_boxes_kernel<7, 4>), dim3(nq), dim3(kSweepThreads), l2, ctx->stream, a);
        else if (a.rp <= 128)
            hipLaunchKernelGGL((sweep_fit_boxes_kernel<8, 4>), dim3(nq), dim3(kSweepThreads), l2, ctx->stream, a);
        else if (a.rp <= 192)
            hipLaunchKernelGGL((sweep_fit_boxes_kernel<12, 1>), dim3(nq), dim3(kSweepThreads), l2, ctx->stream, a);
        else if (a.rp <= 256)
            hipLaunchKernelGGL((sweep_fit_boxes_kernel<16, 1>), dim3(nq), dim3(kSweepThreads), l2, ctx->stream, a);
        else if (a.rp <= 384)
            hipLaunchKernelGGL((sweep_fit_boxes_kernel<24, 1>), dim3(nq), dim3(kSweepThreads), l2, ctx->stream, a);
        else
            hipLaunchKernelGGL((sweep_fit_boxes_kernel<32, 1>), dim3(nq), dim3(kSweepThreads), l2, ctx->stream, a);
        return;
    }
    const int nb = sweep_num_blocks(a.M);
    const size_t lds = (size_t)(2 * a.rp + kGroups * (a.rp > 16 ? a.rp : 16)) * sizeof(double);
    TimerScope ts(ctx, 4);
    if (a.rp <= 128) {
        hipLaunchKernelGGL((sweep_kernel<MODE, 8>), dim3(nb), dim3(kSweepThreads), lds, ctx->stream, a);
    } else {
        if (lds > 48 * 1024)
            set_dynamic_lds(&sweep_kernel<MODE, 32>, (size_t)(lds));
        hipLaunchKernelGGL((sweep_kernel<MODE, 32>), dim3(nb), dim3(kSweepThreads), lds, ctx->stream, a);
    }
    ts.stop();
    if (width > 0 && !a.no_reduce)
        hipLaunchKernelGGL(block_partials_reduce_kernel, dim3((unsigned)width), dim3(256), 0, ctx->stream, a.partial, nb,
                           width, a.out);
}

void launch_sweep(gingr_ctx *ctx, SweepMode mode, const SweepArgs &a) {
    switch (mode) {
        case SWEEP_RHS: launch_sweep_mode<SWEEP_RHS>(ctx, a, a.rp); break;
        case SWEEP_PROJ1: launch_sweep_mode<SWEEP_PROJ1>(ctx, a, a.rp); break;
        case SWEEP_SHAPES: launch_sweep_mode<SWEEP_SHAPES>(ctx, a, 24); break;
        case SWEEP_PROJ2: launch_sweep_mode<SWEEP_PROJ2>(ctx, a, a.rp); break;
        case SWEEP_FIT: launch_sweep_mode<SWEEP_FIT>(ctx, a, 0); break;
        case SWEEP_POSED: launch_sweep_mode<SWEEP_POSED>(ctx, a, 0); break;
        case SWEEP_RHS_ICP: launch_sweep_mode<SWEEP_RHS_ICP>(ctx, a, a.rp); break;
    }
}

static void gram_plan(int64_t M, int32_t rp, int *nbp, int *npatch, int *nslabs, int64_t *rows_per_slab) {
    const int64_t rows = 3 * M;
    *nbp = (rp + 63) / 64;
    *npatch = *nbp * (*nbp + 1) / 2;
    int64_t want = 768 / *npatch;
    if (want < 1) want = 1;
    const int64_t max_slabs = ceil_div(rows, 256);
    if (want > max_slabs) want = max_slabs;
    if (want < 1) want = 1;
    *rows_per_slab = round_up(ceil_div(rows, want), 16);
    *nslabs = (int)ceil_div(rows, *rows_per_slab);
}

static void gram_tri_plan(int64_t M, int *nslabs, int64_t *rows_per_slab) {
    const int64_t rows = 3 * M;
    const int64_t want = std::min<int64_t>(256, std::max<int64_t>(1, ceil_div(rows, 64)));
    *rows_per_slab = round_up(ceil_div(rows, want), 16);
    *nslabs = (int)ceil_div(rows, *rows_per_slab);
}

int64_t gram_ws_doubles(int64_t M, int32_t rp) {
    int nbp, npatch, nslabs, nslabs_tri;
    int64_t rps;
    gram_plan(M, rp, &nbp, &npatch, &nslabs, &rps);
    gram_tri_plan(M, &nslabs_tri, &rps);
    const int64_t n = (int64_t)std::max(nslabs, nslabs_tri) * rp * rp;
    return rp >= 128 ? std::max(n, gram_wide_ws_doubles(M, rp)) : n;
}

int launch_gram(gingr_ctx *ctx, const double *Q0, int64_t M, int32_t rp, const double *weight, double *ws, double *G, const double *evec,
                double *rhs_partial, bool *rhs_done, const ZeroGate *gate) {
    if (rhs_done) *rhs_done = false;
    int nbp, npatch, nslabs;
    int64_t rps;
    gram_plan(M, rp, &nbp, &npatch, &nslabs, &rps);
    {
        const int nt = rp / 16;
        if (nt <= 7) {
            TimerScope ts(ctx, 2);
            gram_tri_plan(M, &nslabs, &rps);
            const bool fuse = evec && rhs_partial && rhs_done;
            if (fuse) *rhs_done = true;
            auto go = [&](auto kern) {
                hipLaunchKernelGGL(kern, dim3(nslabs), dim3(512), 0, ctx->stream, Q0, 3 * M, (int)rp, weight, rps, ws,
                                   fuse ? evec : (const double *)nullptr, M, fuse ? rhs_partial : (double *)nullptr, gate ? *gate : ZeroGate{});
            };
            const bool full = fuse && weight;
#define GINGR_GRAM_TRI(n) \
    case n: \
        if (full) go(gram_tri_kernel<n, true>); \
        else go(gram_tri_kernel<n, false>); \
        break;
            switch (nt) {
                GINGR_GRAM_TRI(1)
                GINGR_GRAM_TRI(2)
                GINGR_GRAM_TRI(3)
                GINGR_GRAM_TRI(4)
                GINGR_GRAM_TRI(5)
                GINGR_GRAM_TRI(6)
                default:
                    if (full) go(gram_tri_kernel<7, true>);
                    else go(gram_tri_kernel<7, false>);
                    break;
            }
#undef GINGR_GRAM_TRI
        } else {
            const bool fuse = evec && rhs_partial && rhs_done;
            if (fuse) *rhs_done = true;
            nslabs = launch_gram_wide(ctx, Q0, M, rp, weight, ws, fuse ? evec : nullptr, fuse ? rhs_partial : nullptr, gate);
        }
    }
    if (G)
        hipLaunchKernelGGL(gram_reduce_kernel, dim3((unsigned)ceil_div((int64_t)rp * rp, 32)), dim3(256), 0, ctx->stream, ws,
                           nslabs, (int)rp, 1, G);
    return nslabs;
}

int launch_gram_downdate(gingr_ctx *ctx, const double *Q0, int64_t M, int32_t rp, const double *weight, double *ws, const ZeroGate *gate) {
    int nslabs_tri;
    int64_t rows_per_slab;
    gram_tri_plan(M, &nslabs_tri, &rows_per_slab);
    const int64_t want = std::max<int64_t>(1, std::min<int64_t>(std::min(nslabs_tri, 128), ceil_div(M, 64)));
    const int64_t vps = ceil_div(M, want);
    const int nslabs = (int)ceil_div(M, vps);
    const int np = (rp + 111) / 112;
    hipLaunchKernelGGL(gram_downdate_kernel, dim3((unsigned)nslabs, (unsigned)(np * (np + 1) / 2)), dim3(256), 0, ctx->stream, Q0, M, (int)rp, weight,
                       vps, ws, gate ? *gate : ZeroGate{});
    return nslabs;
}

void launch_phase1_finalize(gingr_ctx *ctx, const Phase1FinalizeArgs &a) {
    const int nG = (a.nslabs > 0 || a.scaled_src) ? (a.rp * a.rp + 31) / 32 : 0;
    hipLaunchKernelGGL(phase1_finalize_kernel, dim3((unsigned)(nG + a.rp + 1)), dim3(256), 0, ctx->stream, a);
}

namespace {
__global__ __launch_bounds__(256) void moment_scatter_kernel(const double *__restrict__ T, int rp, MomentLayout ml, double *__restrict__ mom) {
    const int64_t idx = (int64_t)blockIdx.x * 256 + threadIdx.x;
    const int64_t w = 3 * (int64_t)rp;
    if (idx >= w * w) return;
    const int I = (int)(idx / w), J = (int)(idx - (int64_t)I * w);
    const int d = I / rp, a = I - d * rp, e = J / rp, b = J - e * rp;
    mom[ml.S(d, e) + (int64_t)a * rp + b] = T[idx];
}
__global__ __launch_bounds__(256) void transpose_kernel(const double *__restrict__ in, int rp, double *__restrict__ out) {
    const int idx = blockIdx.x * 256 + threadIdx.x;
    if (idx >= rp * rp) return;
    const int i = idx / rp, j = idx - i * rp;
    out[idx] = in[j * rp + i];
}
bool moments_as_rows(int32_t rp) { return 3 * rp >= 128 && 3 * rp <= 512; }
}

int64_t moment_grams_ws_doubles(int64_t M, int32_t rp) {
    if (moments_as_rows(rp)) return gram_rows_ws_doubles(M, 3 * rp) + 9 * (int64_t)rp * rp;
    return gram_ws_doubles(M, rp);
}

void launch_moment_grams(gingr_ctx *ctx, const double *Q0, int64_t M, int32_t rp, double *ws, double *mom) {
    const MomentLayout ml{rp};
    if (moments_as_rows(rp)) {
        const int32_t w = 3 * rp;
        double *T = ws + gram_rows_ws_doubles(M, w);
        const int nslabs = launch_gram_rows(ctx, Q0, M, w, ws);
        hipLaunchKernelGGL(gram_reduce_kernel, dim3((unsigned)ceil_div((int64_t)w * w, 32)), dim3(256), 0, ctx->stream, ws, nslabs, (int)w, 1, T);
        hipLaunchKernelGGL(moment_scatter_kernel, dim3((unsigned)ceil_div((int64_t)w * w, 256)), dim3(256), 0, ctx->stream, T, (int)rp, ml, mom);
        return;
    }
    int nbp, npatch, nslabs;
    int64_t rps;
    gram_plan(M, rp, &nbp, &npatch, &nslabs, &rps);
    rps = round_up(ceil_div(M, nslabs), 16);
    nslabs = (int)ceil_div(M, rps);
    for (int d = 0; d < 3; ++d)
        for (int e = d; e < 3; ++e) {
            hipLaunchKernelGGL(gram_kernel, dim3(nslabs, nbp * nbp), dim3(256), 0, ctx->stream, Q0, M, (int)rp, (const double *)nullptr, rps, nbp,
                               3, d, e, 1, ws);
            hipLaunchKernelGGL(gram_reduce_kernel, dim3((unsigned)ceil_div((int64_t)rp * rp, 32)), dim3(256), 0, ctx->stream, ws, nslabs, (int)rp, 0,
                               mom + ml.S(d, e));
            if (e > d)
                hipLaunchKernelGGL(transpose_kernel, dim3((unsigned)ceil_div((int64_t)rp * rp, 256)), dim3(256), 0, ctx->stream, mom + ml.S(d, e),
                                   (int)rp, mom + ml.S(e, d));
        }
}

void launch_centered_mean(gingr_ctx *ctx, const gingr_model *m, double *ptil) {
    hipLaunchKernelGGL(centered_mean_kernel, dim3((unsigned)ceil_div(m->M, 256)), dim3(256), 0, ctx->stream, m->ref, m->mean,
                       m->M, m->c0[0], m->c0[1], m->c0[2], ptil);
}

void launch_obs_cpd(gingr_ctx *ctx, const gingr_model *m, const DevState *st, Cloud fit, const double *P1,
                    const double *PX, double lambda, const int32_t *lm_mask, double *weight, double *evec) {
    hipLaunchKernelGGL(obs_cpd_kernel, dim3((unsigned)ceil_div(m->M, 256)), dim3(256), 0, ctx->stream, m->ref, m->mean, m->M,
                       st, fit, P1, PX, lambda, lm_mask, weight, evec);
}

void launch_obs_icp(gingr_ctx *ctx, const gingr_model *m, const DevState *st, Cloud target, const int32_t *idx,
                    const int32_t *lm_mask, double *weight, double *evec) {
    hipLaunchKernelGGL(obs_points_kernel, dim3((unsigned)ceil_div(m->M, 256)), dim3(256), 0, ctx->stream, m->ref, m->mean,
                       m->M, st, (const double *)nullptr, target, idx, (const double *)nullptr, lm_mask, weight, evec, (int32_t *)nullptr);
}

void launch_obs_points(gingr_ctx *ctx, const gingr_model *m, const DevState *st, const double *obs_soa,
                       const double *weight_in, double *weight, double *evec, const int32_t *lm_mask, int32_t *zero_counts) {
    Cloud none{nullptr, nullptr, nullptr, 0};
    hipLaunchKernelGGL(obs_points_kernel, dim3((unsigned)ceil_div(m->M, 256)), dim3(256), 0, ctx->stream, m->ref, m->mean,
                       m->M, st, obs_soa, none, (const int32_t *)nullptr, weight_in, lm_mask, weight, evec, zero_counts);
}

void launch_landmarks(gingr_ctx *ctx, const gingr_model *m, const DevState *st, int32_t n_lm, const int32_t *lm_pid_local,
                      const double *lm_xyz, const double *lm_cov, double *G, double *rhs) {
    if (n_lm <= 0) return;
    hipLaunchKernelGGL(landmarks_kernel, dim3((unsigned)m->rp + 1), dim3(kLmChunk), 0, ctx->stream, m->Q0, m->ref, m->mean, m->M, (int)m->rp, st,
                       (int)n_lm, lm_pid_local, lm_xyz, lm_cov, G, rhs);
}

int64_t posterior_work_doubles(int32_t rp) {
    const int64_t two_panel_workspaces = (int64_t)lds_solve_doubles(rp, kNB) * (rp >= 128 ? 2 : 1);
    const int64_t two_dense_systems = rp > 240 ? 2 * (round_up(rp, 64) + 64) * round_up(rp, 64) + 2 * (round_up(rp, 64) / 64) * 4096 + 6 * round_up(rp, 64) + 4 : 0;
// ... 33 lines not shown
    }
    __syncthreads();
    if (threadIdx.x == 0) {
        if (*flag == GINGR_ERR_NOT_SPD)
            st->err = GINGR_ERR_NOT_SPD;
        else if (bad)
            st->err = GINGR_ERR_NONFINITE;
    }
}
}

namespace {
__global__ __launch_bounds__(256) void logpdf_system_kernel(int r, int n, int64_t Mp, const double *__restrict__ G, const double *__restrict__ Stot,
                                                            const double *__restrict__ rhs, const double *__restrict__ qte, double *__restrict__ Aw,
                                                            int32_t *__restrict__ flag) {
    const int64_t c = (int64_t)blockIdx.x * 256 + threadIdx.x, row = blockIdx.y;
    if (c == 0 && row == 0) *flag = 0;
    if (c >= Mp) return;
    double v = 0.0;
    if (row < Mp) {
        if (c <= row) {
            if (row < r && c < r) {
                v = __builtin_fma(GINGR_COEFF_NOISE, G[row * n + c], Stot[row * n + c]);
                if (row == c) v += GINGR_COEFF_NOISE;
            } else {
                v = row == c ? 1.0 : 0.0;
            }
        }
    } else if (row == Mp && c < r) {
        v = __builtin_fma(GINGR_COEFF_NOISE, rhs[c], qte[c]);
    }
    Aw[row * Mp + c] = v;
}
__global__ __launch_bounds__(512) void logpdf_finish_kernel(int r, int n, int64_t Mp, const double *__restrict__ G, const double *__restrict__ rhs,
                                                            const double *__restrict__ Wn, const double *__restrict__ Wk, const double *__restrict__ Lk,
                                                            const int32_t *__restrict__ flag_n, const int32_t *__restrict__ flag_k,
                                                            double *__restrict__ fx, double *__restrict__ out2) {
    __shared__ double w[512], hv[2][512], red[512];
    const int tid = threadIdx.x;
    for (int k = tid; k < n; k += 512) w[k] = k < r ? Wk[k] : 0.0;
    __syncthreads();
    for (int kk = tid & 255; kk < r; kk += 256) {
        const int half = tid >> 8;
        const int j0 = half ? (r + 1) / 2 : 0, j1 = half ? r : (r + 1) / 2;
        double s0 = 0.0, s1 = 0.0, s2 = 0.0, s3 = 0.0;
        int j = j0;
        for (; j + 3 < j1; j += 4) {
            s0 = __builtin_fma(G[(int64_t)j * n + kk], w[j], s0);
            s1 = __builtin_fma(G[(int64_t)(j + 1) * n + kk], w[j + 1], s1);
            s2 = __builtin_fma(G[(int64_t)(j + 2) * n + kk], w[j + 2], s2);
            s3 = __builtin_fma(G[(int64_t)(j + 3) * n + kk], w[j + 3], s3);
        }
        for (; j < j1; ++j) s0 = __builtin_fma(G[(int64_t)j * n + kk], w[j], s0);
        hv[half][kk] = (s0 + s1) + (s2 + s3);
    }
    for (int64_t e = tid; e < (int64_t)n * n; e += 512) {
        const int64_t i = e / n, j = e - i * n;
        fx[e] = j <= i ? Lk[i * Mp + j] : 0.0;
    }
    for (int k = tid; k < n; k += 512) {
        fx[(int64_t)n * n + k] = k < r ? Wn[k] : 0.0;
        fx[(int64_t)n * n + n + k] = 1.0 / Lk[(int64_t)k * Mp + k];
    }
    __syncthreads();
    double part = 0.0;
    for (int k = tid; k < r; k += 512) {
        const double nw = (hv[0][k] + hv[1][k]) + w[k];
        part = __builtin_fma(w[k] - Wn[k], nw - rhs[k], part);
    }
    red[tid] = part;
    __syncthreads();
    for (int st2 = 256; st2 > 0; st2 >>= 1) {
        if (tid < st2) red[tid] += red[tid + st2];
        __syncthreads();
    }
    if (tid == 0) {
        const bool bad = *flag_n != 0 || *flag_k != 0;
        out2[0] = bad ? __builtin_nan("") : -0.5 * red[0] - 0.5 * (double)r * 1.8378770664093454836;
        out2[1] = bad ? 1.0 : 0.0;
    }
}
}

void launch_posterior_solve(gingr_ctx *ctx, int32_t r, int32_t rp, const double *G, const double *rhs, const double *zrand,
                            double *work, double *a, DevState *st) {
    TimerScope ts(ctx, 5);
    if (rp > 240 && !zrand) {
        const int64_t Mp = round_up(rp, 64), nb = Mp / 64;
        double *Aw = work, *Linv = Aw + (Mp + 64) * Mp, *W = Linv + nb * 64 * 64;
        int32_t *flag = reinterpret_cast<int32_t *>(W + 3 * Mp);
        hipLaunchKernelGGL(solve_system_kernel, dim3((unsigned)ceil_div(Mp, 256), (unsigned)(Mp + 64)), dim3(256), 0, ctx->stream, (int)r, (int)rp, Mp, G,
                           rhs, Aw, flag);
        dense_spd_solve3(ctx, Aw, Mp, Linv, W, flag);
        hipLaunchKernelGGL(solve_finish_kernel, dim3(1), dim3(256), 0, ctx->stream, (int)r, (int)rp, W, flag, a, st);
        return;
    }
    if (r <= 128) {
        const bool fast = rp <= 112;
        const size_t lds = lds_solve_doubles(rp, fast ? 2 * kNB : kNB) * sizeof(double);
        auto go = [&](auto kern) {
            if (lds > 48 * 1024)
                set_dynamic_lds(kern, (size_t)(lds));
            hipLaunchKernelGGL(kern, dim3(1), dim3(kSolveThreads), lds, ctx->stream, (int)r, (int)rp, G, rhs, zrand, a, st, (double *)nullptr);
        };
        if (fast)
            go(posterior_solve_lds_kernel<0>);
        else
            go(posterior_solve_lds_kernel<1>);
        return;
    }
    auto gow = [&](auto kern, int sw) {
        const size_t lds = (size_t)(rp + kNB) * (sw + 1) * sizeof(double);
        set_dynamic_lds(kern, (size_t)(lds));
        hipLaunchKernelGGL(kern, dim3(1), dim3(kWideSolveThreads), lds, ctx->stream, (int)r, (int)rp, G, rhs, zrand, a, st, work);
    };
    if (rp <= 256)
        gow(posterior_solve_wide_kernel<64>, 64);
    else
        gow(posterior_solve_wide_kernel<32>, 32);
}

namespace {
__global__ __launch_bounds__(1024) void posterior_solve_eig_kernel(int r, int rp, const double *__restrict__ V,
                                                                   const double *__restrict__ lam, const double *__restrict__ sigma2,
                                                                   const double *__restrict__ rhs, double *__restrict__ a, DevState *st) {
    __shared__ double x[512], t[512];
    __shared__ int bad;
    const int tid = threadIdx.x, lane16 = tid & 15, grp = tid >> 4;
    if (tid == 0) bad = 0;
    for (int k = tid; k < r; k += 1024) x[k] = rhs[k];
    __syncthreads();
    const double inv_s2 = 1.0 / sigma2[0];
    for (int k = grp; k < r; k += 64) {
        double s = 0.0;
        for (int i = lane16; i < r; i += 16) s = __builtin_fma(V[(int64_t)i * r + k], x[i], s);
        s = group16_sum(s);
        if (lane16 == 0) t[k] = s / (1.0 + lam[k] * inv_s2);
    }
    __syncthreads();
    for (int i = grp; i < rp; i += 64) {
        double s = 0.0;
        if (i < r)
            for (int k = lane16; k < r; k += 16) s = __builtin_fma(V[(int64_t)i * r + k], t[k], s);
        s = group16_sum(s);
        if (lane16 == 0) {
            a[i] = i < r ? s : 0.0;
            if (!finite_d(s)) bad = 1;
        }
    }
    __syncthreads();
    if (tid == 0 && bad) st->err = GINGR_ERR_NONFINITE;
}
}

void launch_posterior_solve_eig(gingr_ctx *ctx, int32_t r, int32_t rp, const double *eigV, const double *eigL, const double *sigma2,
                                const double *rhs, double *a, DevState *st) {
    hipLaunchKernelGGL(posterior_solve_eig_kernel, dim3(1), dim3(1024), 0, ctx->stream, (int)r, (int)rp, eigV, eigL, sigma2, rhs, a, st);
}

int launch_posterior_logpdf(gingr_ctx *ctx, int32_t r, int32_t rp, const double *G, const double *rhs, const double *Stot,
                            const double *qte, double *fx, bool cached, double *work, double *out2, unsigned *sync, unsigned epoch,
                            bool keep_factor, double *nfac) {
    const size_t lds = lds_solve_doubles(rp, kNB) * sizeof(double);
    const bool in_lds = rp <= 112;
    if (!cached && in_lds && fx && sync) {
        const size_t lds2 = lds_solve_doubles(rp, 2 * kNB) * sizeof(double);
// ... 147 lines not shown
```

include/gingr_hip.h:

```cpp
#ifndef GINGR_HIP_H
#define GINGR_HIP_H

#include <stddef.h>
#include <stdint.h>

#ifdef __cplusplus
extern "C" {
#endif

typedef struct gingr_ctx gingr_ctx;
typedef struct gingr_model gingr_model;
typedef struct gingr_fitter gingr_fitter;

typedef enum gingr_status {
    GINGR_OK = 0,
    GINGR_ERR_BAD_ARGUMENT = 1,
    GINGR_ERR_HIP = 2,
    GINGR_ERR_NONFINITE = 3,
    GINGR_ERR_NOT_SPD = 4,
    GINGR_ERR_NO_DEVICE = 5,
    GINGR_ERR_STATE = 6
} gingr_status;

typedef enum gingr_global_transform {
    GINGR_NO_TRANSFORMS = 0,
    GINGR_RIGID_TRANSFORMS = 1,
    GINGR_SIMILARITY_TRANSFORMS = 2
} gingr_global_transform;

typedef enum gingr_fitting_status {
    GINGR_FIT_NONE = 0,
    GINGR_FIT_CONVERGED = 1,
    GINGR_FIT_MAX_ITERATION = 2,
    GINGR_FIT_MODEL_FLEXIBILITY_ERROR = 3
} gingr_fitting_status;


int gingr_device_count(void);
int gingr_ctx_create(int device, gingr_ctx **out);
void gingr_ctx_destroy(gingr_ctx *ctx);
const char *gingr_last_error(const gingr_ctx *ctx);
int gingr_ctx_set_stream(gingr_ctx *ctx, void *hip_stream);
void *gingr_ctx_get_stream(gingr_ctx *ctx);
int gingr_ctx_synchronize(gingr_ctx *ctx);
const char *gingr_build_info(void);
typedef enum gingr_ctx_option {
    GINGR_OPT_CULL = 0,
    GINGR_OPT_FINE_CULL = 1,
    GINGR_OPT_NN_GRID = 2,
    GINGR_OPT_TRI_GRID = 3,
    GINGR_OPT_SPLIT_EXCHANGE = 4,
    GINGR_OPT_GRAM_DOWNDATE = 5
} gingr_ctx_option;
int gingr_ctx_set_option(gingr_ctx *ctx, int32_t option, int32_t value);
int gingr_ctx_get_option(gingr_ctx *ctx, int32_t option, int32_t *value);


int gingr_cpd_stats(gingr_ctx *ctx, int64_t M, const double *fit, int64_t N, const double *target, double sigma2,
                    double w, double *den, double *P1, double *PX, double *Pt1, double *scalars);

int gingr_cpd_initial_sigma2(gingr_ctx *ctx, int64_t M, const double *ref, int64_t N, const double *target,
                             double *sigma2_out);

int gingr_nn(gingr_ctx *ctx, int64_t M, const double *query, int64_t N, const double *target, int32_t *idx,
             double *d2, double *mean_distance);

int gingr_gauss_block(gingr_ctx *ctx, int64_t na, const double *A, int64_t nb, const double *B, double sigma,
                      double scaling, double *out);

int gingr_model_upload(gingr_ctx *ctx, int64_t M_total, int32_t rank, const double *ref, const double *mean,
                       const double *basis_colmajor, const double *variance, int64_t row_begin, int64_t row_end,
                       gingr_model **out);
void gingr_model_destroy(gingr_model *model);
int gingr_model_gram_exchange(gingr_model *model, void **dev_ptr, int64_t *count);
int gingr_model_finalize(gingr_ctx *ctx, gingr_model *model);
int gingr_gpmm_build_gaussian(gingr_ctx *ctx, int64_t M_total, const double *ref, int32_t n_kernels, const double *sigmas,
                              const double *scalings, double relative_tolerance, int32_t max_rank, int64_t row_begin,
                              int64_t row_end, gingr_model **out);
#define GINGR_KERNEL_GAUSSIAN_MIXTURE 0
#define GINGR_KERNEL_DOT 1
#define GINGR_KERNEL_LOOKUP 2
typedef struct gingr_scalar_kernel {
    int32_t kind;
    int32_t n_kernels;
    const double *sigmas;
    const double *scalings;
    double mirror;
    double scaling;
    const double *lookup;
} gingr_scalar_kernel;
int gingr_gpmm_build_diagonal(gingr_ctx *ctx, int64_t M_total, const double *ref, const gingr_scalar_kernel *kx,
                              const gingr_scalar_kernel *ky, const gingr_scalar_kernel *kz, double relative_tolerance,
                              int32_t max_rank, int64_t row_begin, int64_t row_end, gingr_model **out);
int gingr_pointset_distance_extrema(gingr_ctx *ctx, const double *xyz, int64_t n, double *max_distance, double *min_distance);
int gingr_model_download(gingr_ctx *ctx, const gingr_model *model, double *ref, double *mean, double *basis_colmajor,
                         double *variance);
int64_t gingr_model_num_points(const gingr_model *model);
int32_t gingr_model_rank(const gingr_model *model);

int gingr_model_instance(gingr_ctx *ctx, const gingr_model *model, const double *alpha, const double euler[3],
                         const double center[3], const double translation[3], double scale, double *out_xyz);

int gingr_model_coefficients(gingr_ctx *ctx, const gingr_model *model, const double euler[3], const double center[3],
                             const double translation[3], const double *mesh_xyz, double *alpha);

int gingr_model_posterior_mean(gingr_ctx *ctx, const gingr_model *model, const double euler[3], const double center[3],
                               const double translation[3], const double *obs_xyz, const double *weight,
                               int32_t n_lm, const int32_t *lm_pid, const double *lm_xyz, const double *lm_cov,
                               double *mean_xyz, double *coeffs);

typedef struct gingr_state_scalars {
    double euler[3];
    double center[3];
    double translation[3];
    double scale;
    double sigma2;
    int32_t iteration;
    int32_t status;
} gingr_state_scalars;

typedef struct gingr_cpd_params {
    double w;
    double lambda;
} gingr_cpd_params;

typedef struct gingr_icp_params {
    double initial_sigma;
    double end_sigma;
    int32_t max_iterations;
} gingr_icp_params;

int gingr_fitter_create(gingr_ctx *ctx, const gingr_model *model, gingr_fitter **out);
void gingr_fitter_destroy(gingr_fitter *f);
int gingr_fitter_set_target(gingr_fitter *f, int64_t N, const double *target_xyz);
int gingr_fitter_set_landmarks(gingr_fitter *f, int32_t n_lm, const int32_t *lm_pid, const double *lm_xyz,
// ... 165 lines not shown
```

Measured before the change: 447.9 iterations/s.

## Exploit per-coordinate block structure of GP basis in gram, solve and fit sweep

At model finalize, the code detects whether each basis column touches only one coordinate (x, y or z). If so it packs a compact per-coordinate basis Qc and routes three paths through block versions: the Gram/RHS accumulation, three independent small posterior solves instead of one rank-wide solve, and the fit sweep. This cuts the flops and bytes of the Gram and solve stages when the model is block-separable. It adds detection and packing cost at finalize, extra memory, and only applies when the synthetic model actually has that structure.

```diff
diff --git a/gingr_amd/_native.py b/gingr_amd/_native.py
--- a/gingr_amd/_native.py
+++ b/gingr_amd/_native.py
@@ -65,7 +65,7 @@
 _ip = POINTER(c_int32)
 
 KERNEL_GAUSSIAN_MIXTURE, KERNEL_DOT, KERNEL_LOOKUP = 0, 1, 2
-OPT_CULL, OPT_FINE_CULL, OPT_NN_GRID, OPT_TRI_GRID, OPT_SPLIT_EXCHANGE, OPT_GRAM_DOWNDATE = 0, 1, 2, 3, 4, 5
+OPT_CULL, OPT_FINE_CULL, OPT_NN_GRID, OPT_TRI_GRID, OPT_SPLIT_EXCHANGE, OPT_GRAM_DOWNDATE, OPT_BLOCK_BASIS = 0, 1, 2, 3, 4, 5, 6
 
 
 class ScalarKernel(ctypes.Structure):
diff --git a/gingr_amd/csrc/common.h b/gingr_amd/csrc/common.h
--- a/gingr_amd/csrc/common.h
+++ b/gingr_amd/csrc/common.h
@@ -37,6 +37,7 @@
     void *rccl_comm = nullptr;
     int32_t rccl_world = 0, rccl_rank = 0;
     int split_exchange = 0;
+    int block_basis = 1;
     int gram_downdate = -1;
     hipStream_t side_stream = nullptr, exchange_stream = nullptr;
     hipEvent_t split_ev[2] = {nullptr, nullptr};
diff --git a/gingr_amd/csrc/context.hip b/gingr_amd/csrc/context.hip
--- a/gingr_amd/csrc/context.hip
+++ b/gingr_amd/csrc/context.hip
@@ -153,6 +153,7 @@
         case GINGR_OPT_TRI_GRID: ctx->tri_grid = value < 0 ? 0 : (value > 2 ? 2 : value); return GINGR_OK;
         case GINGR_OPT_SPLIT_EXCHANGE: ctx->split_exchange = value != 0; return GINGR_OK;
         case GINGR_OPT_GRAM_DOWNDATE: ctx->gram_downdate = value < 0 ? -1 : (value != 0); return GINGR_OK;
+        case GINGR_OPT_BLOCK_BASIS: ctx->block_basis = value != 0; return GINGR_OK;
         default: return gingr_set_error(ctx, GINGR_ERR_BAD_ARGUMENT, "ctx_set_option: unknown option %d", option);
     }
 }
@@ -166,6 +167,7 @@
         case GINGR_OPT_TRI_GRID: *value = ctx->tri_grid; return GINGR_OK;
         case GINGR_OPT_SPLIT_EXCHANGE: *value = ctx->split_exchange; return GINGR_OK;
         case GINGR_OPT_GRAM_DOWNDATE: *value = ctx->gram_downdate; return GINGR_OK;
+        case GINGR_OPT_BLOCK_BASIS: *value = ctx->block_basis; return GINGR_OK;
         default: return gingr_set_error(ctx, GINGR_ERR_BAD_ARGUMENT, "ctx_get_option: unknown option %d", option);
     }
 }
diff --git a/gingr_amd/csrc/fitter.hip b/gingr_amd/csrc/fitter.hip
--- a/gingr_amd/csrc/fitter.hip
+++ b/gingr_amd/csrc/fitter.hip
@@ -327,11 +327,19 @@
     f->fit_boxes_valid = true;
 }
 
+bool blocks_on(const gingr_fitter *f) { return f->m->blk && f->ctx->block_basis; }
+bool cpd_blocks(const gingr_fitter *f) { return blocks_on(f) && f->m->M == f->m->M_total && !f->partial_out; }
+
 void refresh_fit(gingr_fitter *f) {
     SweepArgs a = base_args(f);
     a.coef0 = f->alpha;
     a.shape_out = f->fit;
     if (f->fboxes && f->m->rp <= 512 && f->cpd_seen) {
+        if (blocks_on(f)) {
+            a.Q0 = f->m->Qc;
+            a.rp = f->m->kp;
+            a.blk_cols = f->m->blk_cols;
+        }
         a.qboxes = f->fboxes + 6 * ceil_div(f->m->M, 256);
         a.box_centre = f->absmax + 2;
         a.absmax_slot = f->absmax + 1;
@@ -375,6 +383,69 @@
     f->Tm = f->Tt = 0;
 }
 
+void detect_blocks(gingr_ctx *ctx, gingr_model *m) {
+    dev_free(m->Qc);
+    dev_free(m->blk_cols);
+    dev_free(m->blk_map);
+    m->Qc = nullptr, m->blk_cols = m->blk_map = nullptr;
+    m->blk = false;
+    m->kp = 0, m->kd[0] = m->kd[1] = m->kd[2] = 0;
+    const int r = m->r, rp = m->rp;
+    DevBuf flags;
+    if (flags.alloc((size_t)3 * rp * sizeof(int32_t)) != hipSuccess) return (void)hipGetLastError();
+    (void)hipMemsetAsync(flags.p, 0, (size_t)3 * rp * sizeof(int32_t), ctx->stream);
+    launch_basis_coord_flags(ctx, m->Q0, m->M, rp, flags.as<int32_t>());
+    std::vector<int32_t> hf((size_t)3 * rp);
+    std::vector<double> sdiag((size_t)3 * r);
+    const MomentLayout ml{rp};
+    bool ok = hipMemcpyAsync(hf.data(), flags.p, hf.size() * sizeof(int32_t), hipMemcpyDeviceToHost, ctx->stream) == hipSuccess;
+    for (int d = 0; d < 3 && ok; ++d)
+        ok = hipMemcpy2DAsync(sdiag.data() + (size_t)d * r, sizeof(double), m->mom + ml.S(d, d), (size_t)(rp + 1) * sizeof(double),
+                              sizeof(double), (size_t)r, hipMemcpyDeviceToHost, ctx->stream) == hipSuccess;
+    if (!ok || hipStreamSynchronize(ctx->stream) != hipSuccess) return (void)hipGetLastError();
+    std::vector<int32_t> owner((size_t)r, -1);
+    int kd[3] = {0, 0, 0};
+    for (int k = 0; k < r; ++k) {
+        for (int d = 0; d < 3; ++d) {
+            const double v = sdiag[(size_t)d * r + k];
+            if (v != 0.0 || v != v) {
+                if (owner[(size_t)k] >= 0) return;
+                owner[(size_t)k] = d;
+            }
+        }
+        for (int d = 0; d < 3; ++d)
+            if (hf[(size_t)d * rp + k] && owner[(size_t)k] != d) return;
+        if (owner[(size_t)k] >= 0) ++kd[owner[(size_t)k]];
+    }
+    const int kp = (int)round_up(std::max(std::max(kd[0], kd[1]), std::max(kd[2], 1)), 16);
+    if (kp > 112) return;
+    std::vector<int32_t> cols((size_t)3 * kp, -1), map((size_t)rp, -1);
+    int fill[3] = {0, 0, 0};
+    for (int k = 0; k < r; ++k) {
+        const int d = owner[(size_t)k];
+        if (d < 0) continue;
+        cols[(size_t)d * kp + fill[d]] = k;
+        map[(size_t)k] = d * kp + fill[d];
+        ++fill[d];
+    }
+    if (dev_alloc(ctx, &m->Qc, (size_t)(3 * m->M + kBasisRowSlack) * kp) || dev_alloc(ctx, &m->blk_cols, cols.size()) ||
+        dev_alloc(ctx, &m->blk_map, map.size()) ||
+        hipMemcpy(m->blk_cols, cols.data(), cols.size() * sizeof(int32_t), hipMemcpyHostToDevice) != hipSuccess ||
+        hipMemcpy(m->blk_map, map.data(), map.size() * sizeof(int32_t), hipMemcpyHostToDevice) != hipSuccess) {
+        (void)hipGetLastError();
+        dev_free(m->Qc);
+        dev_free(m->blk_cols);
+        dev_free(m->blk_map);
+        m->Qc = nullptr, m->blk_cols = m->blk_map = nullptr;
+        return;
+    }
+    launch_pack_blocks(ctx, m->Q0, m->M, rp, kp, m->blk_cols, m->Qc);
+    if (hipStreamSynchronize(ctx->stream) != hipSuccess) return (void)hipGetLastError();
+    m->kp = kp;
+    for (int d = 0; d < 3; ++d) m->kd[d] = kd[d];
+    m->blk = true;
+}
+
 int model_finalize_impl(gingr_ctx *ctx, gingr_model *m) {
     DevBuf work, flag;
     HIP_TRY(ctx, work.alloc((size_t)binv_work_doubles(m->rp) * sizeof(double)));
@@ -416,6 +487,7 @@
             (void)hipGetLastError();
     }
     HIP_TRY(ctx, hipStreamSynchronize(ctx->stream));
+    detect_blocks(ctx, m);
     m->finalized = true;
     return GINGR_OK;
 }
@@ -585,6 +657,9 @@
     dev_free(m->pvec);
     dev_free(m->perm);
     dev_free(m->iperm);
+    dev_free(m->Qc);
+    dev_free(m->blk_cols);
+    dev_free(m->blk_map);
     delete m;
 }
 
@@ -1467,7 +1542,16 @@
                 }
             } else {
                 fa.gram_partial = gram_ws;
-                fa.nslabs = launch_gram(ctx, m->Q0, M, rp, f->weight, gram_ws, nullptr, f->evec, sweep_ws, &rhs_done);
+                if (!icp && cpd_blocks(f))
+                    fa.nslabs = launch_gram_blocks(ctx, m->Qc, M, m->kp, f->weight, f->evec, gram_ws, gram_ws_doubles(M, rp), sweep_ws,
+                                                   sweep_ws_doubles(M, rp));
+                if (fa.nslabs > 0) {
+                    fa.blk_map = m->blk_map;
+                    fa.blk_kp = m->kp;
+                    rhs_done = true;
+                } else {
+                    fa.nslabs = launch_gram(ctx, m->Q0, M, rp, f->weight, gram_ws, nullptr, f->evec, sweep_ws, &rhs_done);
+                }
             }
             fa.sweep_partial = sweep_ws;
             if (rhs_done) {
@@ -1501,6 +1585,9 @@
                 launch_posterior_solve_eig(ctx, r, rp, m->eigV, m->eigL, &f->st->sigma2, rhs, f->acoef, f->st);
             else if (f->zrand_active && f->allow_alt && f->post_stage == 2 && f->nf_valid[f->live] && m->M == m->M_total && !f->partial_out)
                 launch_posterior_sample_cached(ctx, r, rp, f->nfac[f->live], f->fxbuf[f->live] + (int64_t)rp * rp, f->zrand, f->acoef, f->st);
+            else if (!icp && f->n_lm == 0 && !f->zrand_active && cpd_blocks(f) &&
+                     posterior_solve_blocks_work_doubles(m->kp) <= (int64_t)rp * rp)
+                launch_posterior_solve_blocks(ctx, m, G, rhs, f->work, f->acoef, f->st);
             else
                 launch_posterior_solve(ctx, r, rp, G, rhs, f->zrand_active ? f->zrand : nullptr, f->work, f->acoef, f->st);
             launch_post_matvecs(ctx, m, f->alpha, f->acoef, f->zbuf);
diff --git a/gingr_amd/csrc/gp.h b/gingr_amd/csrc/gp.h
--- a/gingr_amd/csrc/gp.h
+++ b/gingr_amd/csrc/gp.h
@@ -98,6 +98,10 @@
     double Ps[3] = {0};
     std::vector<double> variance;
     bool finalized = false;
+    bool blk = false;
+    int32_t kp = 0, kd[3] = {0, 0, 0};
+    double *Qc = nullptr;
+    int32_t *blk_cols = nullptr, *blk_map = nullptr;
 };
 
 void launch_interp_pack(gingr_ctx *ctx, const double *Qs, int32_t rp, const int32_t *inv_src, const int32_t *ids, const double *w,
@@ -187,6 +191,7 @@
     double *weight_out, *evec_out;
     const DevState *frame;
     ZeroGate gate;
+    const int32_t *blk_cols;
 };
 
 int sweep_num_blocks(int64_t M);
@@ -222,10 +227,21 @@
     int32_t contribute_xpx;
     ZeroGate gate;
     int32_t alt_nslabs;
+    const int32_t *blk_map;
+    int32_t blk_kp;
 };
 void launch_phase1_finalize(gingr_ctx *ctx, const Phase1FinalizeArgs &a);
 int launch_gram_downdate(gingr_ctx *ctx, const double *Q0, int64_t M, int32_t rp, const double *weight, double *ws,
                          const ZeroGate *gate = nullptr);
+
+void launch_basis_coord_flags(gingr_ctx *ctx, const double *Q0, int64_t M, int32_t rp, int32_t *flags);
+void launch_pack_blocks(gingr_ctx *ctx, const double *Q0, int64_t M, int32_t rp, int32_t kp, const int32_t *blk_cols, double *Qc);
+int launch_gram_blocks(gingr_ctx *ctx, const double *Qc, int64_t M, int32_t kp, const double *weight, const double *evec, double *ws,
+                       int64_t ws_cap, double *rhs_partial, int64_t rhs_cap);
+
+int64_t posterior_solve_blocks_work_doubles(int32_t kp);
+void launch_posterior_solve_blocks(gingr_ctx *ctx, const gingr_model *m, const double *G, const double *rhs, double *work, double *a,
+                                   DevState *st);
 
 void launch_obs_cpd(gingr_ctx *ctx, const gingr_model *m, const DevState *st, Cloud fit, const double *P1,
                     const double *PX, double lambda, const int32_t *lm_mask, double *weight, double *evec);
diff --git a/gingr_amd/csrc/gp.hip b/gingr_amd/csrc/gp.hip
--- a/gingr_amd/csrc/gp.hip
+++ b/gingr_amd/csrc/gp.hip
@@ -262,16 +262,24 @@
     if (threadIdx.x == 0) out[k] = sh[0];
 }
 
-template <int KM, int S>
+template <int KM, int S, bool BLK = false>
 __global__ __launch_bounds__(kSweepThreads) void sweep_fit_boxes_kernel(SweepArgs a) {
     constexpr int CH = KM < 8 ? KM : 8;
+    constexpr int NC = BLK ? 3 : 1;
     static_assert(4 % S == 0, "points per group and round");
     extern __shared__ double lds[];
     const int tid = threadIdx.x, lane16 = tid & 15, grp = tid >> 4;
     const int rp = a.rp, km = rp >> 4;
     const int64_t M = a.M;
-    double *coef = lds, *red = lds + rp;
-    for (int k = tid; k < rp; k += kSweepThreads) coef[k] = a.coef0[k];
+    double *coef = lds, *red = lds + NC * rp;
+    if constexpr (BLK) {
+        for (int k = tid; k < 3 * rp; k += kSweepThreads) {
+            const int c = a.blk_cols[k];
+            coef[k] = c >= 0 ? a.coef0[c] : 0.0;
+        }
+    } else {
+        for (int k = tid; k < rp; k += kSweepThreads) coef[k] = a.coef0[k];
+    }
     double R[9], tr[3], cen[3];
     for (int q = 0; q < 9; ++q) R[q] = a.state->R[q];
     for (int q = 0; q < 3; ++q) {
@@ -279,10 +287,12 @@
         cen[q] = a.state->center[q];
     }
     const double scale = a.state->scale;
-    double cf[KM];
-    __syncthreads();
-#pragma unroll
-    for (int m = 0; m < KM; ++m) cf[m] = m < km ? coef[m * 16 + lane16] : 0.0;
+    double cf[NC][KM];
+    __syncthreads();
+#pragma unroll
+    for (int c = 0; c < NC; ++c)
+#pragma unroll
+        for (int m = 0; m < KM; ++m) cf[c][m] = m < km ? coef[c * rp + m * 16 + lane16] : 0.0;
     double amax = 0.0;
     for (int64_t qd = blockIdx.x; qd * 64 < M; qd += gridDim.x) {
         double lo[3] = {__builtin_huge_val(), __builtin_huge_val(), __builtin_huge_val()};
@@ -315,7 +325,7 @@
                     for (int d = 0; d < 3; ++d)
 #pragma unroll
                         for (int m = 0; m < CH; ++m)
-                            if (mc + m < KM) facc[s][d] = __builtin_fma(u[s][d][m], cf[mc + m], facc[s][d]);
+                            if (mc + m < KM) facc[s][d] = __builtin_fma(u[s][d][m], cf[BLK ? d : 0][mc + m], facc[s][d]);
             }
 #pragma unroll
             for (int s = 0; s < S; ++s) {
@@ -486,7 +496,7 @@
     return t + q;
 }
 
-template <int NT, int HALF, bool FULL>
+template <int NT, int HALF, bool FULL, bool PL = false>
 __device__ __forceinline__ void gram_tri_half(const double *__restrict__ Q0, int rp, const double *__restrict__ weight, int64_t r0,
                                               int64_t r1, int kgroup, int kq, int cl, int lane, double *red, double *xchg,
                                               double *__restrict__ out, const double *__restrict__ evec, int64_t npts,
@@ -504,18 +514,19 @@
     const int kgu = __builtin_amdgcn_readfirstlane(kgroup);
     const int64_t ubase = r0 + 4 * kgu;
     const int64_t first = ubase + kq;
-    const double *pclamp = Q0 + r0 * rp + cl;
-    const double *pnext = Q0 + first * rp + cl;
-    const int64_t pstep = 16 * (int64_t)rp;
+    const int64_t pitch = PL ? 3 * (int64_t)rp : rp;
+    const double *pclamp = Q0 + r0 * pitch + cl;
+    const double *pnext = Q0 + first * pitch + cl;
+    const int64_t pstep = 16 * pitch;
     int64_t left_u = r1 - ubase;
     const int64_t pt_first = first / 3;
     const int rem_first = (int)(first - 3 * pt_first);
     constexpr unsigned kThird = 0x55555556u;
     unsigned third = (unsigned)rem_first * kThird;
-    const double *wclamp = with_w ? weight + r0 / 3 : pclamp;
-    const double *eclamp = with_rhs ? evec + r0 / 3 : pclamp;
-    const double *wp = with_w ? weight + pt_first : pclamp;
-    const double *ep = with_rhs ? evec + rem_first * npts + pt_first : pclamp;
+    const double *wclamp = with_w ? weight + (PL ? r0 : r0 / 3) : pclamp;
+    const double *eclamp = with_rhs ? evec + (PL ? r0 : r0 / 3) : pclamp;
+    const double *wp = with_w ? weight + (PL ? first : pt_first) : pclamp;
+    const double *ep = with_rhs ? evec + (PL ? first : rem_first * npts + pt_first) : pclamp;
     const int64_t estep = with_rhs ? 5 + npts : 0, ewrap = with_rhs ? 6 - 2 * npts : 0;
     double fn[2][kO], wn[2], en[2];
     int vrows[2];
@@ -538,11 +549,16 @@
         }
         left_u -= 16;
         pnext += pstep;
-        const unsigned t2 = third + kThird;
-        const bool wrap = t2 < third;
-        third = t2;
-        wp += wrap ? 6 : 5;
-        ep += wrap ? ewrap : estep;
+        if constexpr (PL) {
+            wp += 16;
+            ep += 16;
+        } else {
+            const unsigned t2 = third + kThird;
+            const bool wrap = t2 < third;
+            third = t2;
+            wp += wrap ? 6 : 5;
+            ep += wrap ? ewrap : estep;
+        }
     };
     double racc[kO];
 #pragma unroll
@@ -671,7 +687,7 @@
                 for (int reg = 0; reg < 4; ++reg) out[(int64_t)(16 * t + kq + 4 * reg) * rp + 16 * u + cl] = acc[q >> 1][reg];
 }
 
-template <int NT, bool FULL>
+template <int NT, bool FULL, bool PL = false>
 __global__ __launch_bounds__(512) void gram_tri_kernel(const double *__restrict__ Q0, int64_t rows, int rp,
                                                        const double *__restrict__ weight, int64_t rows_per_slab,
                                                        double *__restrict__ partial, const double *__restrict__ evec, int64_t npts,
@@ -684,12 +700,16 @@
     const int wave = threadIdx.x >> 6, lane = threadIdx.x & 63, kq = lane >> 4, cl = lane & 15;
     const int64_t r0 = (int64_t)blockIdx.x * rows_per_slab;
     const int64_t r1 = min(rows, r0 + rows_per_slab);
-    double *out = partial + (int64_t)blockIdx.x * rp * rp;
-    double *rhs_out = rhs_partial ? rhs_partial + (int64_t)blockIdx.x * rp : nullptr;
+    const int d = PL ? (int)blockIdx.y : 0;
+    const int64_t slab = PL ? (int64_t)blockIdx.x * 3 + d : (int64_t)blockIdx.x;
+    const double *Qb = Q0 + (PL ? d * rp : 0);
+    const double *eb = (PL && evec) ? evec + d * npts : evec;
+    double *out = partial + slab * rp * rp;
+    double *rhs_out = rhs_partial ? rhs_partial + slab * rp : nullptr;
     if ((wave >> 2) == 0)
-        gram_tri_half<NT, 0, FULL>(Q0, rp, weight, r0, r1, wave & 3, kq, cl, lane, red, xchg, out, evec, npts, rhs_out, rsh);
+        gram_tri_half<NT, 0, FULL, PL>(Qb, rp, weight, r0, r1, wave & 3, kq, cl, lane, red, xchg, out, eb, npts, rhs_out, rsh);
     else
-        gram_tri_half<NT, 1, FULL>(Q0, rp, weight, r0, r1, wave & 3, kq, cl, lane, red, xchg, out, evec, npts, rhs_out, rsh);
+        gram_tri_half<NT, 1, FULL, PL>(Qb, rp, weight, r0, r1, wave & 3, kq, cl, lane, red, xchg, out, eb, npts, rhs_out, rsh);
 }
 
 __global__ __launch_bounds__(256) void gram_reduce_kernel(const double *__restrict__ partial, int nslabs, int rp, int symmetric,
@@ -725,6 +745,47 @@
         A.nslabs = A.alt_nslabs;
         A.scaled_src = nullptr;
         A.sweep_blocks = A.alt_nslabs;
+    }
+    if (A.blk_map) {
+        const int kp = A.blk_kp, kk = kp * kp;
+        if (b < nG) {
+            const int el = threadIdx.x & 31, g = threadIdx.x >> 5;
+            const int idx = b * 32 + el;
+            const int i = idx / rp, j = idx - i * rp;
+            const int mi = idx < rr ? A.blk_map[i] : -1, mj = idx < rr ? A.blk_map[j] : -1;
+            const bool same = mi >= 0 && mj >= 0 && mi / kp == mj / kp;
+            double s = 0.0;
+            if (same && i <= j) {
+                const int dd = mi / kp;
+                const double *p = A.gram_partial + (int64_t)dd * kk + (int64_t)(mi - dd * kp) * kp + (mj - dd * kp);
+#pragma unroll 8
+                for (int q = g; q < A.nslabs; q += 8) s += p[(int64_t)q * 3 * kk];
+            }
+            sh[g][el] = s;
+            __syncthreads();
+            if (g == 0 && idx < rr && i <= j) {
+                const double t = ((sh[0][el] + sh[1][el]) + (sh[2][el] + sh[3][el])) + ((sh[4][el] + sh[5][el]) + (sh[6][el] + sh[7][el]));
+                A.G[i * rp + j] = same ? t : 0.0;
+                A.G[j * rp + i] = same ? t : 0.0;
+            }
+            return;
+        }
+        if (b < nG + rp) {
+            const int k = b - nG;
+            const int mk = A.blk_map[k];
+            double s = 0.0;
+            if (mk >= 0)
+                for (int q = threadIdx.x; q < A.sweep_blocks; q += 256) s += A.sweep_partial[(int64_t)q * 3 * kp + mk];
+            sv[threadIdx.x] = s;
+            __syncthreads();
+#pragma unroll
+            for (int st = 128; st > 0; st >>= 1) {
+                if ((int)threadIdx.x < st) sv[threadIdx.x] += sv[threadIdx.x + st];
+                __syncthreads();
+            }
+            if (threadIdx.x == 0) A.rhs[k] = sv[0];
+            return;
+        }
     }
     if (b < nG) {
         const int el = threadIdx.x & 31, g = threadIdx.x >> 5;
@@ -1524,6 +1585,38 @@
 #endif
 }
 
+__global__ __launch_bounds__(kSolveThreads) void posterior_solve_blocks_kernel(int r, int rp, int kp, int n0, int n1, int n2,
+                                                                          const int32_t *__restrict__ blk_cols,
+                                                                          const int32_t *__restrict__ blk_map,
+                                                                          const double *__restrict__ G, const double *__restrict__ rhs,
+                                                                          double *__restrict__ work, double *__restrict__ a,
+                                                                          DevState *__restrict__ st) {
+    extern __shared__ double lds_sm[];
+    __shared__ int bad_spd, bad;
+    const int d = blockIdx.x, tid = threadIdx.x;
+    const int n = d == 0 ? n0 : (d == 1 ? n1 : n2);
+    const int32_t *cols = blk_cols + d * kp;
+    const int64_t kk = (int64_t)kp * kp;
+    double *Gd = work + d * kk;
+    double *rd = work + 3 * kk + d * kp;
+    double *xd = work + 3 * kk + 3 * kp + d * kp;
+    DevState *sd = reinterpret_cast<DevState *>(work + 3 * kk + 6 * kp) + d;
+    if (d == 0)
+        for (int k = tid; k < rp; k += kSolveThreads)
+            if (k >= r || blk_map[k] < 0) a[k] = 0.0;
+    if (n == 0) return;
+    for (int e = tid; e < kk; e += kSolveThreads) {
+        const int i = e / kp, j = e - i * kp;
+        Gd[e] = (i < n && j < n) ? G[(int64_t)cols[i] * rp + cols[j]] : 0.0;
+    }
+    for (int j = tid; j < kp; j += kSolveThreads) rd[j] = j < n ? rhs[cols[j]] : 0.0;
+    __syncthreads();
+    posterior_solve_body<true>(lds_sm, n, kp, Gd, rd, nullptr, xd, sd, &bad_spd, &bad);
+    __syncthreads();
+    for (int j = tid; j < n; j += kSolveThreads) a[cols[j]] = xd[j];
+    if (tid == 0 && (bad_spd || bad)) atomicMax(&st->err, bad_spd ? (int32_t)GINGR_ERR_NOT_SPD : (int32_t)GINGR_ERR_NONFINITE);
+}
+
 constexpr int kWideSolveThreads = 512;
 
 template <int SW>
@@ -2567,9 +2660,14 @@
 static void launch_sweep_mode(gingr_ctx *ctx, const SweepArgs &a, int width) {
     if (MODE == SWEEP_FIT && a.qboxes && a.rp <= 512) {
         const int nq = (int)std::min<int64_t>(4096, ceil_div(a.M, 64));
-        const size_t l2 = (size_t)(a.rp + kGroups * 8 + 8) * sizeof(double);
+        const size_t l2 = (size_t)((a.blk_cols ? 3 : 1) * a.rp + kGroups * 8 + 8) * sizeof(double);
         TimerScope ts(ctx, 4);
-        if (a.rp <= 64)
+        if (a.blk_cols) {
+            if (a.rp <= 64)
+                hipLaunchKernelGGL((sweep_fit_boxes_kernel<4, 4, true>), dim3(nq), dim3(kSweepThreads), l2, ctx->stream, a);
+            else
+                hipLaunchKernelGGL((sweep_fit_boxes_kernel<7, 1, true>), dim3(nq), dim3(kSweepThreads), l2, ctx->stream, a);
+        } else if (a.rp <= 64)
             hipLaunchKernelGGL((sweep_fit_boxes_kernel<4, 4>), dim3(nq), dim3(kSweepThreads), l2, ctx->stream, a);
         else if (a.rp <= 112)
             hipLaunchKernelGGL((sweep_fit_boxes_kernel<7, 4>), dim3(nq), dim3(kSweepThreads), l2, ctx->stream, a);
@@ -2709,6 +2807,77 @@
 }
 
 namespace {
+__global__ __launch_bounds__(256) void basis_coord_flags_kernel(const double *__restrict__ Q0, int64_t M, int rp, int32_t *__restrict__ flags) {
+    __shared__ int32_t sf[3 * 512];
+    for (int k = threadIdx.x; k < 3 * rp; k += 256) sf[k] = 0;
+    __syncthreads();
+    const int64_t n = 3 * M * (int64_t)rp;
+    for (int64_t e = (int64_t)blockIdx.x * 256 + threadIdx.x; e < n; e += (int64_t)gridDim.x * 256) {
+        if (Q0[e] != 0.0 || Q0[e] != Q0[e]) {
+            const int64_t row = e / rp;
+            const int k = (int)(e - row * rp), dd = (int)(row % 3);
+            if (!sf[dd * rp + k]) atomicOr(&sf[dd * rp + k], 1);
+        }
+    }
+    __syncthreads();
+    for (int k = threadIdx.x; k < 3 * rp; k += 256)
+        if (sf[k]) atomicOr(&flags[k], 1);
+}
+
+__global__ __launch_bounds__(256) void pack_blocks_kernel(const double *__restrict__ Q0, int64_t M, int rp, int kp,
+                                                          const int32_t *__restrict__ cols, double *__restrict__ Qc) {
+    const int64_t n = (3 * M + kBasisRowSlack) * (int64_t)kp;
+    for (int64_t e = (int64_t)blockIdx.x * 256 + threadIdx.x; e < n; e += (int64_t)gridDim.x * 256) {
+        const int64_t row = e / kp;
+        const int j = (int)(e - row * kp);
+        double v = 0.0;
+        if (row < 3 * M) {
+            const int c = cols[(int)(row % 3) * kp + j];
+            if (c >= 0) v = Q0[row * rp + c];
+        }
+        Qc[e] = v;
+    }
+}
+
+}
+
+void launch_basis_coord_flags(gingr_ctx *ctx, const double *Q0, int64_t M, int32_t rp, int32_t *flags) {
+    const int64_t n = 3 * M * (int64_t)rp;
+    const int nb = (int)std::max<int64_t>(1, std::min<int64_t>(2048, ceil_div(n, 256)));
+    hipLaunchKernelGGL(basis_coord_flags_kernel, dim3(nb), dim3(256), 0, ctx->stream, Q0, M, (int)rp, flags);
+}
+
+void launch_pack_blocks(gingr_ctx *ctx, const double *Q0, int64_t M, int32_t rp, int32_t kp, const int32_t *blk_cols, double *Qc) {
+    const int64_t n = (3 * M + kBasisRowSlack) * (int64_t)kp;
+    const int nb = (int)std::max<int64_t>(1, std::min<int64_t>(8192, ceil_div(n, 256)));
+    hipLaunchKernelGGL(pack_blocks_kernel, dim3(nb), dim3(256), 0, ctx->stream, Q0, M, (int)rp, (int)kp, blk_cols, Qc);
+}
+
+int launch_gram_blocks(gingr_ctx *ctx, const double *Qc, int64_t M, int32_t kp, const double *weight, const double *evec, double *ws,
+                       int64_t ws_cap, double *rhs_partial, int64_t rhs_cap) {
+    const int nt = kp / 16;
+    if (nt < 1 || nt > 7 || kp != nt * 16 || !weight || !evec) return 0;
+    const int64_t want = std::min<int64_t>(85, std::max<int64_t>(1, ceil_div(M, 64)));
+    const int64_t rps = round_up(ceil_div(M, want), 16);
+    const int nslabs = (int)ceil_div(M, rps);
+    if ((int64_t)nslabs * 3 * kp * kp > ws_cap || (int64_t)nslabs * 3 * kp > rhs_cap) return 0;
+    TimerScope ts(ctx, 2);
+    auto go = [&](auto kern) {
+        hipLaunchKernelGGL(kern, dim3(nslabs, 3), dim3(512), 0, ctx->stream, Qc, M, (int)kp, weight, rps, ws, evec, M, rhs_partial, ZeroGate{});
+    };
+    switch (nt) {
+        case 1: go(gram_tri_kernel<1, true, true>); break;
+        case 2: go(gram_tri_kernel<2, true, true>); break;
+        case 3: go(gram_tri_kernel<3, true, true>); break;
+        case 4: go(gram_tri_kernel<4, true, true>); break;
+        case 5: go(gram_tri_kernel<5, true, true>); break;
+        case 6: go(gram_tri_kernel<6, true, true>); break;
+        default: go(gram_tri_kernel<7, true, true>); break;
+    }
+    return nslabs;
+}
+
+namespace {
 __global__ __launch_bounds__(256) void moment_scatter_kernel(const double *__restrict__ T, int rp, MomentLayout ml, double *__restrict__ mom) {
     const int64_t idx = (int64_t)blockIdx.x * 256 + threadIdx.x;
     const int64_t w = 3 * (int64_t)rp;
@@ -2908,6 +3077,19 @@
 }
 }
 
+int64_t posterior_solve_blocks_work_doubles(int32_t kp) {
+    return 3 * (int64_t)kp * kp + 6 * (int64_t)kp + 3 * (int64_t)((sizeof(DevState) + 7) / 8);
+}
+
+void launch_posterior_solve_blocks(gingr_ctx *ctx, const gingr_model *m, const double *G, const double *rhs, double *work, double *a,
+                                   DevState *st) {
+    TimerScope ts(ctx, 5);
+    const size_t lds = lds_solve_doubles(m->kp, 2 * kNB) * sizeof(double);
+    if (lds > 48 * 1024) set_dynamic_lds(posterior_solve_blocks_kernel, lds);
+    hipLaunchKernelGGL(posterior_solve_blocks_kernel, dim3(3), dim3(kSolveThreads), lds, ctx->stream, (int)m->r, (int)m->rp, (int)m->kp,
+                       (int)m->kd[0], (int)m->kd[1], (int)m->kd[2], m->blk_cols, m->blk_map, G, rhs, work, a, st);
+}
+
 void launch_posterior_solve(gingr_ctx *ctx, int32_t r, int32_t rp, const double *G, const double *rhs, const double *zrand,
                             double *work, double *a, DevState *st) {
     TimerScope ts(ctx, 5);
diff --git a/include/gingr_hip.h b/include/gingr_hip.h
--- a/include/gingr_hip.h
+++ b/include/gingr_hip.h
@@ -50,7 +50,8 @@
     GINGR_OPT_NN_GRID = 2,
     GINGR_OPT_TRI_GRID = 3,
     GINGR_OPT_SPLIT_EXCHANGE = 4,
-    GINGR_OPT_GRAM_DOWNDATE = 5
+    GINGR_OPT_GRAM_DOWNDATE = 5,
+    GINGR_OPT_BLOCK_BASIS = 6
 } gingr_ctx_option;
 int gingr_ctx_set_option(gingr_ctx *ctx, int32_t option, int32_t value);
 int gingr_ctx_get_option(gingr_ctx *ctx, int32_t option, int32_t *value);
```

New measurement: 459.4 iterations/s, median of 6. +2.6%, better.
